# Gancheekim/ATM-VFI

Hardware: AMD Instinct MI355X
Metric: interpolated frames/s at 1080p (network_base, bs=1) (higher is better)
Workload: dtype f32 (contractions as fp16 hi/lo split x3 MFMA, fp32 accumulate; ~22 significand bits)

## Files before the change

### atm-vfi_amd/csrc/api.hip

```cpp
#include "common.h"

#include <string.h>

#include <vector>

namespace atmvfi {

static thread_local char g_err[512] = "";

void set_error(const char* fmt, ...) {
    va_list ap;
    va_start(ap, fmt);
    vsnprintf(g_err, sizeof(g_err), fmt, ap);
    va_end(ap);
}

int check_launch(const char* what) {
    const hipError_t e = hipGetLastError();
    if (e != hipSuccess) {
        set_error("%s: launch failed: %s", what, hipGetErrorString(e));
        return ATMVFI_ELAUNCH;
    }
    return ATMVFI_OK;
}

#ifdef ATMVFI_RANGE_CHECK
static std::vector<RangeWordSetter>& range_registry() {
    static std::vector<RangeWordSetter> v;
    return v;
}
void range_registry_add(RangeWordSetter s) { range_registry().push_back(s); }
#endif

}

extern "C" int atmvfi_range_word_set(uint32_t* word, void* stream) {
#ifdef ATMVFI_RANGE_CHECK
    for (atmvfi::RangeWordSetter set : atmvfi::range_registry()) {
        const int e = set(reinterpret_cast<unsigned*>(word), (hipStream_t)stream);
        ATMVFI_REQUIRE(e == 0, ATMVFI_ELAUNCH, "range_word_set: hipMemcpyToSymbolAsync failed (%d)", e);
    }
    return ATMVFI_OK;
#else
    (void)word; (void)stream;
    atmvfi::set_error("range_word_set: this is the default build; the operand range check lives in libatmvfi_hip_checked.so (make checked)");
    return ATMVFI_EINVAL;
#endif
}
extern "C" int atmvfi_range_checked(void) {
#ifdef ATMVFI_RANGE_CHECK
    return 1;
#else
    return 0;
#endif
}

extern "C" int atmvfi_version(void) { return (0 << 16) | (21 << 8) | 0; }
extern "C" const char* atmvfi_last_error(void) { return atmvfi::g_err; }
#ifndef ATMVFI_SOURCE_DIGEST
#define ATMVFI_SOURCE_DIGEST "unknown (api.hip compiled outside the Makefile)"
#endif
extern "C" const char* atmvfi_source_digest(void) { return ATMVFI_SOURCE_DIGEST; }
```

### atm-vfi_amd/csrc/plan_dispatch.inc

```
#define ATMVFI_PLAN_NFN 65
static const char* const kPlanFnNames[ATMVFI_PLAN_NFN] = {
    "atmvfi_conv2d",
    "atmvfi_conv3x3_f16x3",
    "atmvfi_conv3x3_planes",
    "atmvfi_conv3x3_planes2",
    "atmvfi_conv3x3_planes3",
    "atmvfi_conv3x3_planes_readout",
    "atmvfi_deconv2x2",
    "atmvfi_dwconv3x3_gelu",
    "atmvfi_ensemble_select",
    "atmvfi_f32_to_yuv420p10",
    "atmvfi_final_residual",
    "atmvfi_flow_warp",
    "atmvfi_flow_warp_ex",
    "atmvfi_flow_warp_nhwc",
    "atmvfi_flow_warp_tiled",
    "atmvfi_flow_warp_up2",
    "atmvfi_flow_warp_up2_tiled",
    "atmvfi_frame_borders",
    "atmvfi_frame_compose",
    "atmvfi_frame_difference",
    "atmvfi_frame_f32_to_u8",
    "atmvfi_frame_rot180",
    "atmvfi_frame_signature",
    "atmvfi_frame_u8_to_f32",
    "atmvfi_frame_u8_window",
    "atmvfi_gemm",
    "atmvfi_head1x1_planes",
    "atmvfi_image_pyramid",
    "atmvfi_image_pyramid_pack",
    "atmvfi_l1_mean",
    "atmvfi_layernorm",
    "atmvfi_linear",
    "atmvfi_motion_head",
    "atmvfi_motion_head_planes",
    "atmvfi_pack_dw_weight",
    "atmvfi_pack_frames",
    "atmvfi_pack_weight",
    "atmvfi_pack_weight_conv3x3",
    "atmvfi_pack_weight_split",
    "atmvfi_pool_blocks",
    "atmvfi_range_word_set",
    "atmvfi_refine_tail",
    "atmvfi_resize_bilinear_ac",
    "atmvfi_rgb_to_yuv420",
    "atmvfi_shutter_accumulate",
    "atmvfi_shutter_resolve",
    "atmvfi_split_planes",
    "atmvfi_split_planes_at",
    "atmvfi_ssim_psnr",
    "atmvfi_stem_fused",
    "atmvfi_tta_merge",
    "atmvfi_warp_blend",
    "atmvfi_warp_blend_planes",
    "atmvfi_warp_blend_tiled",
    "atmvfi_window_attention",
    "atmvfi_window_attention_f16x3",
    "atmvfi_window_attn_cross_motion",
    "atmvfi_window_attn_self",
    "atmvfi_yuv420_to_rgb",
    "atmvfi_yuv420_window",
    "atmvfi_yuv420p10_to_f32",
    "atmvfi_yuv_sub_decode",
    "atmvfi_yuv_sub_encode",
    "atmvfi_yuv_surface_decode",
    "atmvfi_yuv_surface_encode",
};
static const int kPlanFnArgs[ATMVFI_PLAN_NFN] = {1, 19, 21, 25, 27, 15, 1, 13, 13, 10, 8, 10, 9, 14, 10, 8, 8, 7, 15, 12, 9, 5, 11, 9, 15, 1, 10, 8, 9, 7, 14, 1, 12, 17, 3, 6, 7, 5, 8, 8, 1, 10, 13, 13, 13, 7, 8, 10, 18, 21, 11, 19, 23, 23, 13, 13, 9, 8, 14, 18, 14, 25, 17, 24, 16};
static int plan_call(const atmvfi_plan_op* op, void* stream) {
    const atmvfi_plan_arg* a = op->a;
    switch (op->fn) {
    case 0: return atmvfi_conv2d((const atmvfi_gemm_params*)(uintptr_t)a[0].u, stream);
    case 1: return atmvfi_conv3x3_f16x3((const float*)(uintptr_t)a[0].u, (int)a[1].i, (int)a[2].i, (int)a[3].i, (int)a[4].i, (int)a[5].i, (const void*)(uintptr_t)a[6].u, (const void*)(uintptr_t)a[7].u, (int)a[8].i, (float*)(uintptr_t)a[9].u, (int)a[10].i, (const float*)(uintptr_t)a[11].u, (const float*)(uintptr_t)a[12].u, (void*)(uintptr_t)a[13].u, (void*)(uintptr_t)a[14].u, (int64_t)a[15].i, (const float*)(uintptr_t)a[16].u, (int)a[17].i, (int)a[18].i, stream);
    case 2: return atmvfi_conv3x3_planes((const void*)(uintptr_t)a[0].u, (const void*)(uintptr_t)a[1].u, (int64_t)a[2].i, (int)a[3].i, (int)a[4].i, (int)a[5].i, (int)a[6].i, (const void*)(uintptr_t)a[7].u, (const void*)(uintptr_t)a[8].u, (int)a[9].i, (float*)(uintptr_t)a[10].u, (int)a[11].i, (const float*)(uintptr_t)a[12].u, (const float*)(uintptr_t)a[13].u, (void*)(uintptr_t)a[14].u, (void*)(uintptr_t)a[15].u, (int64_t)a[16].i, (int)a[17].i, (const float*)(uintptr_t)a[18].u, (int)a[19].i, (int)a[20].i, stream);
    case 3: return atmvfi_conv3x3_planes2((const void*)(uintptr_t)a[0].u, (const void*)(uintptr_t)a[1].u, (int64_t)a[2].i, (int)a[3].i, (int)a[4].i, (int)a[5].i, (int)a[6].i, (const void*)(uintptr_t)a[7].u, (const void*)(uintptr_t)a[8].u, (int)a[9].i, (float*)(uintptr_t)a[10].u, (int)a[11].i, (const float*)(uintptr_t)a[12].u, (const float*)(uintptr_t)a[13].u, (void*)(uintptr_t)a[14].u, (void*)(uintptr_t)a[15].u, (int64_t)a[16].i, (int)a[17].i, (const float*)(uintptr_t)a[18].u, (void*)(uintptr_t)a[19].u, (void*)(uintptr_t)a[20].u, (int64_t)a[21].i, (int)a[22].i, (int)a[23].i, (int)a[24].i, stream);
    case 4: return atmvfi_conv3x3_planes3((const void*)(uintptr_t)a[0].u, (const void*)(uintptr_t)a[1].u, (int64_t)a[2].i, (int)a[3].i, (int)a[4].i, (int)a[5].i, (int)a[6].i, (const void*)(uintptr_t)a[7].u, (const void*)(uintptr_t)a[8].u, (int)a[9].i, (float*)(uintptr_t)a[10].u, (int)a[11].i, (const float*)(uintptr_t)a[12].u, (const float*)(uintptr_t)a[13].u, (void*)(uintptr_t)a[14].u, (void*)(uintptr_t)a[15].u, (int64_t)a[16].i, (int)a[17].i, (const float*)(uintptr_t)a[18].u, (void*)(uintptr_t)a[19].u, (void*)(uintptr_t)a[20].u, (int64_t)a[21].i, (int)a[22].i, (int)a[23].i, (int)a[24].i, (float*)(uintptr_t)a[25].u, (int64_t)a[26].i, stream);
    case 5: return atmvfi_conv3x3_planes_readout((const void*)(uintptr_t)a[0].u, (const void*)(uintptr_t)a[1].u, (int64_t)a[2].i, (int)a[3].i, (int)a[4].i, (int)a[5].i, (int)a[6].i, (const void*)(uintptr_t)a[7].u, (const void*)(uintptr_t)a[8].u, (int)a[9].i, (const float*)(uintptr_t)a[10].u, (const float*)(uintptr_t)a[11].u, (const void*)(uintptr_t)a[12].u, (float*)(uintptr_t)a[13].u, (int64_t)a[14].i, stream);
    case 6: return atmvfi_deconv2x2((const atmvfi_gemm_params*)(uintptr_t)a[0].u, stream);
    case 7: return atmvfi_dwconv3x3_gelu((const float*)(uintptr_t)a[0].u, (int)a[1].i, (float*)(uintptr_t)a[2].u, (int)a[3].i, (const float*)(uintptr_t)a[4].u, (const float*)(uintptr_t)a[5].u, (int)a[6].i, (int)a[7].i, (int)a[8].i, (int)a[9].i, (void*)(uintptr_t)a[10].u, (void*)(uintptr_t)a[11].u, (int)a[12].i, stream);
    case 8: return atmvfi_ensemble_select((const float*)(uintptr_t)a[0].u, (const float*)(uintptr_t)a[1].u, (const float*)(uintptr_t)a[2].u, (const float*)(uintptr_t)a[3].u, (const float*)(uintptr_t)a[4].u, (const float*)(uintptr_t)a[5].u, (const float*)(uintptr_t)a[6].u, (const float*)(uintptr_t)a[7].u, (const float*)(uintptr_t)a[8].u, (float*)(uintptr_t)a[9].u, (float*)(uintptr_t)a[10].u, (int)a[11].i, (int64_t)a[12].i, stream);
    case 9: return atmvfi_f32_to_yuv420p10((const float*)(uintptr_t)a[0].u, (int)a[1].i, (int)a[2].i, (int)a[3].i, (int)a[4].i, (int)a[5].i, (int)a[6].i, (int)a[7].i, (int)a[8].i, (void*)(uintptr_t)a[9].u, stream);
    case 10: return atmvfi_final_residual((const float*)(uintptr_t)a[0].u, (const float*)(uintptr_t)a[1].u, (int)a[2].i, (float*)(uintptr_t)a[3].u, (float*)(uintptr_t)a[4].u, (int)a[5].i, (int)a[6].i, (int)a[7].i, stream);
    case 11: return atmvfi_flow_warp((const float*)(uintptr_t)a[0].u, (const float*)(uintptr_t)a[1].u, (int64_t)a[2].i, (int)a[3].i, (int)a[4].i, (float*)(uintptr_t)a[5].u, (int)a[6].i, (int)a[7].i, (int)a[8].i, (int)a[9].i, stream);
    case 12: return atmvfi_flow_warp_ex((const float*)(uintptr_t)a[0].u, (const float*)(uintptr_t)a[1].u, (float*)(uintptr_t)a[2].u, (uint8_t*)(uintptr_t)a[3].u, (int)a[4].i, (int)a[5].i, (int)a[6].i, (int)a[7].i, (int)a[8].i, stream);
    case 13: return atmvfi_flow_warp_nhwc((const float*)(uintptr_t)a[0].u, (int)a[1].i, (int64_t)a[2].i, (const float*)(uintptr_t)a[3].u, (int64_t)a[4].i, (int)a[5].i, (int)a[6].i, (float*)(uintptr_t)a[7].u, (int)a[8].i, (int64_t)a[9].i, (int)a[10].i, (int)a[11].i, (int)a[12].i, (int)a[13].i, stream);
    case 14: return atmvfi_flow_warp_tiled((const float*)(uintptr_t)a[0].u, (const float*)(uintptr_t)a[1].u, (int64_t)a[2].i, (int)a[3].i, (int)a[4].i, (float*)(uintptr_t)a[5].u, (int)a[6].i, (int)a[7].i, (int)a[8].i, (int)a[9].i, stream);
    case 15: return atmvfi_flow_warp_up2((const float*)(uintptr_t)a[0].u, (const float*)(uintptr_t)a[1].u, (float*)(uintptr_t)a[2].u, (float*)(uintptr_t)a[3].u, (int)a[4].i, (int)a[5].i, (int)a[6].i, (int)a[7].i, stream);
    case 16: return atmvfi_flow_warp_up2_tiled((const float*)(uintptr_t)a[0].u, (const float*)(uintptr_t)a[1].u, (float*)(uintptr_t)a[2].u, (float*)(uintptr_t)a[3].u, (int)a[4].i, (int)a[5].i, (int)a[6].i, (int)a[7].i, stream);
    case 17: return atmvfi_frame_borders((const void*)(uintptr_t)a[0].u, (int)a[1].i, (int)a[2].i, (int)a[3].i, (int32_t*)(uintptr_t)a[4].u, (int32_t*)(uintptr_t)a[5].u, (int64_t)a[6].i, stream);
    case 18: return atmvfi_frame_compose((void*)(uintptr_t)a[0].u, (const void*)(uintptr_t)a[1].u, (int)a[2].i, (int)a[3].i, (int)a[4].i, (int)a[5].i, (int)a[6].i, (int)a[7].i, (const float*)(uintptr_t)a[8].u, (int)a[9].i, (int)a[10].i, (int)a[11].i, (int)a[12].i, (const void*)(uintptr_t)a[13].u, (int)a[14].i, stream);
    case 19: return atmvfi_frame_difference((const void*)(uintptr_t)a[0].u, (const void*)(uintptr_t)a[1].u, (int)a[2].i, (int)a[3].i, (int)a[4].i, (int)a[5].i, (int)a[6].i, (int)a[7].i, (int)a[8].i, (int32_t*)(uintptr_t)a[9].u, (int32_t*)(uintptr_t)a[10].u, (int64_t)a[11].i, stream);
    case 20: return atmvfi_frame_f32_to_u8((const float*)(uintptr_t)a[0].u, (int)a[1].i, (int)a[2].i, (int)a[3].i, (int)a[4].i, (void*)(uintptr_t)a[5].u, (int)a[6].i, (int)a[7].i, (int)a[8].i, stream);
    case 21: return atmvfi_frame_rot180((const float*)(uintptr_t)a[0].u, (float*)(uintptr_t)a[1].u, (int)a[2].i, (int)a[3].i, (int)a[4].i, stream);
    case 22: return atmvfi_frame_signature((const void*)(uintptr_t)a[0].u, (int)a[1].i, (int)a[2].i, (int)a[3].i, (int)a[4].i, (int)a[5].i, (int)a[6].i, (int)a[7].i, (int32_t*)(uintptr_t)a[8].u, (int32_t*)(uintptr_t)a[9].u, (int64_t)a[10].i, stream);
    case 23: return atmvfi_frame_u8_to_f32((const void*)(uintptr_t)a[0].u, (int)a[1].i, (int)a[2].i, (int)a[3].i, (float*)(uintptr_t)a[4].u, (int)a[5].i, (int)a[6].i, (int)a[7].i, (int)a[8].i, stream);
    case 24: return atmvfi_frame_u8_window((const void*)(uintptr_t)a[0].u, (int)a[1].i, (int)a[2].i, (int)a[3].i, (int)a[4].i, (int)a[5].i, (int)a[6].i, (int)a[7].i, (int)a[8].i, (float*)(uintptr_t)a[9].u, (int)a[10].i, (int)a[11].i, (int)a[12].i, (int)a[13].i, (void*)(uintptr_t)a[14].u, stream);
    case 25: return atmvfi_gemm((const atmvfi_gemm_params*)(uintptr_t)a[0].u, stream);
    case 26: return atmvfi_head1x1_planes((const void*)(uintptr_t)a[0].u, (const void*)(uintptr_t)a[1].u, (int64_t)a[2].i, (int64_t)a[3].i, (int)a[4].i, (const float*)(uintptr_t)a[5].u, (const float*)(uintptr_t)a[6].u, (int)a[7].i, (float*)(uintptr_t)a[8].u, (int)a[9].i, stream);
    case 27: return atmvfi_image_pyramid((const float*)(uintptr_t)a[0].u, (const float*)(uintptr_t)a[1].u, (float*)(uintptr_t)a[2].u, (float*)(uintptr_t)a[3].u, (float*)(uintptr_t)a[4].u, (int)a[5].i, (int)a[6].i, (int)a[7].i, stream);
    case 28: return atmvfi_image_pyramid_pack((const float*)(uintptr_t)a[0].u, (const float*)(uintptr_t)a[1].u, (float*)(uintptr_t)a[2].u, (float*)(uintptr_t)a[3].u, (float*)(uintptr_t)a[4].u, (float*)(uintptr_t)a[5].u, (int)a[6].i, (int)a[7].i, (int)a[8].i, stream);
    case 29: return atmvfi_l1_mean((const float*)(uintptr_t)a[0].u, (const float*)(uintptr_t)a[1].u, (float*)(uintptr_t)a[2].u, (int)a[3].i, (int64_t)a[4].i, (float*)(uintptr_t)a[5].u, (int64_t)a[6].i, stream);
    case 30: return atmvfi_layernorm((const float*)(uintptr_t)a[0].u, (int)a[1].i, (int64_t)a[2].i, (int)a[3].i, (const int32_t*)(uintptr_t)a[4].u, (float*)(uintptr_t)a[5].u, (int)a[6].i, (const float*)(uintptr_t)a[7].u, (const float*)(uintptr_t)a[8].u, (int64_t)a[9].i, (int)a[10].i, (void*)(uintptr_t)a[11].u, (void*)(uintptr_t)a[12].u, (int)a[13].i, stream);
    case 31: return atmvfi_linear((const atmvfi_gemm_params*)(uintptr_t)a[0].u, stream);
    case 32: return atmvfi_motion_head((const float*)(uintptr_t)a[0].u, (const int32_t*)(uintptr_t)a[1].u, (const float*)(uintptr_t)a[2].u, (const float*)(uintptr_t)a[3].u, (const float*)(uintptr_t)a[4].u, (const float*)(uintptr_t)a[5].u, (float*)(uintptr_t)a[6].u, (int)a[7].i, (int64_t)a[8].i, (int)a[9].i, (int64_t)a[10].i, (int)a[11].i, stream);
    case 33: return atmvfi_motion_head_planes((const float*)(uintptr_t)a[0].u, (const int32_t*)(uintptr_t)a[1].u, (const float*)(uintptr_t)a[2].u, (const float*)(uintptr_t)a[3].u, (const float*)(uintptr_t)a[4].u, (const float*)(uintptr_t)a[5].u, (float*)(uintptr_t)a[6].u, (int)a[7].i, (int64_t)a[8].i, (int)a[9].i, (int64_t)a[10].i, (int)a[11].i, (void*)(uintptr_t)a[12].u, (void*)(uintptr_t)a[13].u, (int64_t)a[14].i, (int)a[15].i, (int)a[16].i, stream);
    case 34: return atmvfi_pack_dw_weight((const float*)(uintptr_t)a[0].u, (float*)(uintptr_t)a[1].u, (int)a[2].i, stream);
    case 35: return atmvfi_pack_frames((const float*)(uintptr_t)a[0].u, (const float*)(uintptr_t)a[1].u, (float*)(uintptr_t)a[2].u, (int)a[3].i, (int)a[4].i, (int)a[5].i, stream);
    case 36: return atmvfi_pack_weight((int)a[0].i, (const float*)(uintptr_t)a[1].u, (float*)(uintptr_t)a[2].u, (int)a[3].i, (int)a[4].i, (int)a[5].i, (int)a[6].i, stream);
    case 37: return atmvfi_pack_weight_conv3x3((const float*)(uintptr_t)a[0].u, (void*)(uintptr_t)a[1].u, (void*)(uintptr_t)a[2].u, (int)a[3].i, (int)a[4].i, stream);
    case 38: return atmvfi_pack_weight_split((int)a[0].i, (const float*)(uintptr_t)a[1].u, (void*)(uintptr_t)a[2].u, (void*)(uintptr_t)a[3].u, (int)a[4].i, (int)a[5].i, (int)a[6].i, (int)a[7].i, stream);
    case 39: return atmvfi_pool_blocks((void*)(uintptr_t)a[0].u, (int64_t)a[1].i, (int)a[2].i, (const int32_t*)(uintptr_t)a[3].u, (int)a[4].i, (int64_t)a[5].i, (void*)(uintptr_t)a[6].u, (int)a[7].i, stream);
    case 40: return atmvfi_range_word_set((uint32_t*)(uintptr_t)a[0].u, stream);
    case 41: return atmvfi_refine_tail((const float*)(uintptr_t)a[0].u, (int64_t)a[1].i, (const float*)(uintptr_t)a[2].u, (const float*)(uintptr_t)a[3].u, (const float*)(uintptr_t)a[4].u, (float*)(uintptr_t)a[5].u, (float*)(uintptr_t)a[6].u, (int)a[7].i, (int)a[8].i, (int)a[9].i, stream);
    case 42: return atmvfi_resize_bilinear_ac((const float*)(uintptr_t)a[0].u, (int64_t)a[1].i, (int64_t)a[2].i, (int64_t)a[3].i, (int64_t)a[4].i, (float*)(uintptr_t)a[5].u, (int)a[6].i, (int)a[7].i, (int)a[8].i, (int)a[9].i, (int)a[10].i, (int)a[11].i, (float)a[12].f, stream);
    case 43: return atmvfi_rgb_to_yuv420((const void*)(uintptr_t)a[0].u, (int)a[1].i, (const float*)(uintptr_t)a[2].u, (int)a[3].i, (int)a[4].i, (int)a[5].i, (int)a[6].i, (int)a[7].i, (int)a[8].i, (int)a[9].i, (int)a[10].i, (int)a[11].i, (void*)(uintptr_t)a[12].u, stream);
    case 44: return atmvfi_shutter_accumulate((int32_t*)(uintptr_t)a[0].u, (int)a[1].i, (int)a[2].i, (const float*)(uintptr_t)a[3].u, (int)a[4].i, (int)a[5].i, (int)a[6].i, (int)a[7].i, (const uint8_t*)(uintptr_t)a[8].u, (int)a[9].i, (int)a[10].i, (int)a[11].i, (int)a[12].i, stream);
    case 45: return atmvfi_shutter_resolve((const int32_t*)(uintptr_t)a[0].u, (int)a[1].i, (int)a[2].i, (int)a[3].i, (int)a[4].i, (uint8_t*)(uintptr_t)a[5].u, (int)a[6].i, stream);
    case 46: return atmvfi_split_planes((const float*)(uintptr_t)a[0].u, (int)a[1].i, (int64_t)a[2].i, (int)a[3].i, (const float*)(uintptr_t)a[4].u, (void*)(uintptr_t)a[5].u, (void*)(uintptr_t)a[6].u, (int)a[7].i, stream);
    case 47: return atmvfi_split_planes_at((const float*)(uintptr_t)a[0].u, (int)a[1].i, (int64_t)a[2].i, (int)a[3].i, (const float*)(uintptr_t)a[4].u, (void*)(uintptr_t)a[5].u, (void*)(uintptr_t)a[6].u, (int)a[7].i, (int)a[8].i, (int)a[9].i, stream);
    case 48: return atmvfi_ssim_psnr((const void*)(uintptr_t)a[0].u, (int64_t)a[1].i, (int64_t)a[2].i, (int64_t)a[3].i, (int64_t)a[4].i, (const float*)(uintptr_t)a[5].u, (int64_t)a[6].i, (int64_t)a[7].i, (int64_t)a[8].i, (int64_t)a[9].i, (int)a[10].i, (int)a[11].i, (int)a[12].i, (float)a[13].f, (int)a[14].i, (double*)(uintptr_t)a[15].u, (float*)(uintptr_t)a[16].u, (int64_t)a[17].i, stream);
    case 49: return atmvfi_stem_fused((const float*)(uintptr_t)a[0].u, (int)a[1].i, (int)a[2].i, (int)a[3].i, (int)a[4].i, (int)a[5].i, (const void*)(uintptr_t)a[6].u, (const void*)(uintptr_t)a[7].u, (const float*)(uintptr_t)a[8].u, (const float*)(uintptr_t)a[9].u, (const void*)(uintptr_t)a[10].u, (const void*)(uintptr_t)a[11].u, (const float*)(uintptr_t)a[12].u, (const float*)(uintptr_t)a[13].u, (const void*)(uintptr_t)a[14].u, (const void*)(uintptr_t)a[15].u, (const float*)(uintptr_t)a[16].u, (const float*)(uintptr_t)a[17].u, (void*)(uintptr_t)a[18].u, (void*)(uintptr_t)a[19].u, (int64_t)a[20].i, stream);
    case 50: return atmvfi_tta_merge((const float*)(uintptr_t)a[0].u, (const float*)(uintptr_t)a[1].u, (float*)(uintptr_t)a[2].u, (void*)(uintptr_t)a[3].u, (int)a[4].i, (int)a[5].i, (int)a[6].i, (int)a[7].i, (int)a[8].i, (int)a[9].i, (int)a[10].i, stream);
    case 51: return atmvfi_warp_blend((const float*)(uintptr_t)a[0].u, (const float*)(uintptr_t)a[1].u, (const float*)(uintptr_t)a[2].u, (int)a[3].i, (int64_t)a[4].i, (float*)(uintptr_t)a[5].u, (float*)(uintptr_t)a[6].u, (float*)(uintptr_t)a[7].u, (float*)(uintptr_t)a[8].u, (float*)(uintptr_t)a[9].u, (float*)(uintptr_t)a[10].u, (float*)(uintptr_t)a[11].u, (const float*)(uintptr_t)a[12].u, (const float*)(uintptr_t)a[13].u, (float*)(uintptr_t)a[14].u, (int)a[15].i, (int)a[16].i, (int)a[17].i, (int)a[18].i, stream);
    case 52: return atmvfi_warp_blend_planes((const float*)(uintptr_t)a[0].u, (const float*)(uintptr_t)a[1].u, (const float*)(uintptr_t)a[2].u, (int)a[3].i, (int64_t)a[4].i, (float*)(uintptr_t)a[5].u, (float*)(uintptr_t)a[6].u, (float*)(uintptr_t)a[7].u, (float*)(uintptr_t)a[8].u, (float*)(uintptr_t)a[9].u, (float*)(uintptr_t)a[10].u, (float*)(uintptr_t)a[11].u, (const float*)(uintptr_t)a[12].u, (const float*)(uintptr_t)a[13].u, (float*)(uintptr_t)a[14].u, (int)a[15].i, (void*)(uintptr_t)a[16].u, (void*)(uintptr_t)a[17].u, (int64_t)a[18].i, (int)a[19].i, (int)a[20].i, (int)a[21].i, (int)a[22].i, stream);
    case 53: return atmvfi_warp_blend_tiled((const float*)(uintptr_t)a[0].u, (const float*)(uintptr_t)a[1].u, (const float*)(uintptr_t)a[2].u, (int)a[3].i, (int64_t)a[4].i, (float*)(uintptr_t)a[5].u, (float*)(uintptr_t)a[6].u, (float*)(uintptr_t)a[7].u, (float*)(uintptr_t)a[8].u, (float*)(uintptr_t)a[9].u, (float*)(uintptr_t)a[10].u, (float*)(uintptr_t)a[11].u, (const float*)(uintptr_t)a[12].u, (const float*)(uintptr_t)a[13].u, (float*)(uintptr_t)a[14].u, (int)a[15].i, (void*)(uintptr_t)a[16].u, (void*)(uintptr_t)a[17].u, (int64_t)a[18].i, (int)a[19].i, (int)a[20].i, (int)a[21].i, (int)a[22].i, stream);
    case 54: return atmvfi_window_attention((const float*)(uintptr_t)a[0].u, (float*)(uintptr_t)a[1].u, (float*)(uintptr_t)a[2].u, (const int32_t*)(uintptr_t)a[3].u, (int)a[4].i, (int)a[5].i, (int)a[6].i, (int)a[7].i, (int)a[8].i, (int)a[9].i, (void*)(uintptr_t)a[10].u, (void*)(uintptr_t)a[11].u, (int)a[12].i, stream);
    case 55: return atmvfi_window_attention_f16x3((const float*)(uintptr_t)a[0].u, (float*)(uintptr_t)a[1].u, (float*)(uintptr_t)a[2].u, (const int32_t*)(uintptr_t)a[3].u, (int)a[4].i, (int)a[5].i, (int)a[6].i, (int)a[7].i, (int)a[8].i, (int)a[9].i, (void*)(uintptr_t)a[10].u, (void*)(uintptr_t)a[11].u, (int)a[12].i, stream);
    case 56: return atmvfi_window_attn_cross_motion((const float*)(uintptr_t)a[0].u, (float*)(uintptr_t)a[1].u, (float*)(uintptr_t)a[2].u, (const int32_t*)(uintptr_t)a[3].u, (int)a[4].i, (int)a[5].i, (int)a[6].i, (int)a[7].i, (int)a[8].i, stream);
    case 57: return atmvfi_window_attn_self((const float*)(uintptr_t)a[0].u, (float*)(uintptr_t)a[1].u, (const int32_t*)(uintptr_t)a[2].u, (int)a[3].i, (int)a[4].i, (int)a[5].i, (int)a[6].i, (int)a[7].i, stream);
    case 58: return atmvfi_yuv420_to_rgb((const void*)(uintptr_t)a[0].u, (int)a[1].i, (int)a[2].i, (int)a[3].i, (int)a[4].i, (int)a[5].i, (int)a[6].i, (void*)(uintptr_t)a[7].u, (int)a[8].i, (float*)(uintptr_t)a[9].u, (int)a[10].i, (int)a[11].i, (int)a[12].i, (int)a[13].i, stream);
    case 59: return atmvfi_yuv420_window((const void*)(uintptr_t)a[0].u, (int)a[1].i, (int)a[2].i, (int)a[3].i, (int)a[4].i, (int)a[5].i, (int)a[6].i, (int)a[7].i, (int)a[8].i, (int)a[9].i, (int)a[10].i, (int)a[11].i, (float*)(uintptr_t)a[12].u, (int)a[13].i, (int)a[14].i, (int)a[15].i, (int)a[16].i, (void*)(uintptr_t)a[17].u, stream);
    case 60: return atmvfi_yuv420p10_to_f32((const void*)(uintptr_t)a[0].u, (int)a[1].i, (int)a[2].i, (int)a[3].i, (int)a[4].i, (int)a[5].i, (int)a[6].i, (int)a[7].i, (int)a[8].i, (float*)(uintptr_t)a[9].u, (int)a[10].i, (int)a[11].i, (int)a[12].i, (int)a[13].i, stream);
    case 61: return atmvfi_yuv_sub_decode((const void*)(uintptr_t)a[0].u, (int)a[1].i, (int)a[2].i, (int)a[3].i, (int)a[4].i, (int)a[5].i, (int)a[6].i, (int)a[7].i, (int)a[8].i, (int)a[9].i, (int64_t)a[10].i, (int64_t)a[11].i, (int64_t)a[12].i, (int)a[13].i, (int)a[14].i, (int)a[15].i, (int)a[16].i, (int)a[17].i, (void*)(uintptr_t)a[18].u, (int)a[19].i, (float*)(uintptr_t)a[20].u, (int)a[21].i, (int)a[22].i, (int)a[23].i, (int)a[24].i, stream);
    case 62: return atmvfi_yuv_sub_encode((const void*)(uintptr_t)a[0].u, (int)a[1].i, (const float*)(uintptr_t)a[2].u, (int)a[3].i, (int)a[4].i, (int)a[5].i, (int)a[6].i, (int)a[7].i, (int)a[8].i, (int)a[9].i, (int)a[10].i, (int)a[11].i, (int)a[12].i, (int)a[13].i, (int)a[14].i, (int)a[15].i, (void*)(uintptr_t)a[16].u, stream);
    case 63: return atmvfi_yuv_surface_decode((const void*)(uintptr_t)a[0].u, (int)a[1].i, (int)a[2].i, (int)a[3].i, (int)a[4].i, (int)a[5].i, (int)a[6].i, (int)a[7].i, (int)a[8].i, (int64_t)a[9].i, (int64_t)a[10].i, (int64_t)a[11].i, (int)a[12].i, (int)a[13].i, (int)a[14].i, (int)a[15].i, (int)a[16].i, (void*)(uintptr_t)a[17].u, (int)a[18].i, (float*)(uintptr_t)a[19].u, (int)a[20].i, (int)a[21].i, (int)a[22].i, (int)a[23].i, stream);
    case 64: return atmvfi_yuv_surface_encode((const void*)(uintptr_t)a[0].u, (int)a[1].i, (const float*)(uintptr_t)a[2].u, (int)a[3].i, (int)a[4].i, (int)a[5].i, (int)a[6].i, (int)a[7].i, (int)a[8].i, (int)a[9].i, (int)a[10].i, (int)a[11].i, (int)a[12].i, (int)a[13].i, (int)a[14].i, (void*)(uintptr_t)a[15].u, stream);
    default: break;
    }
    atmvfi::set_error("plan_run: unknown function id %d", op->fn);
    return ATMVFI_EINVAL;
}
```

### atm-vfi_amd/hip_ops.py

```python
from __future__ import annotations

import ctypes
import os
from dataclasses import dataclass
from typing import List, Optional

import torch

from .pixfmt import Surface, _not_420, _origin_error, as_surface

_HERE = os.path.dirname(os.path.abspath(__file__))
LIB_PATH = os.path.join(_HERE, "libatmvfi_hip.so")
CHECKED_LIB_PATH = os.path.join(_HERE, "libatmvfi_hip_checked.so")

GEMM_CONV, GEMM_LINEAR, GEMM_DECONV = 0, 1, 2

c_f = ctypes.c_void_p
c_i = ctypes.c_int
C_SLOTS = ctypes.POINTER(ctypes.c_int32)
c_l = ctypes.c_int64


class HipLibraryMissing(RuntimeError):
    pass


class GemmParams(ctypes.Structure):
    _fields_ = [
        ("mode", ctypes.c_int32),
        ("in_", c_f), ("in_ld", ctypes.c_int32), ("N", ctypes.c_int32), ("H", ctypes.c_int32),
        ("W", ctypes.c_int32), ("Cin", ctypes.c_int32),
        ("in_gstride", ctypes.c_int64), ("in_rpg", ctypes.c_int32),
        ("weight", c_f),
        ("Cout", ctypes.c_int32), ("kh", ctypes.c_int32), ("kw", ctypes.c_int32), ("stride", ctypes.c_int32),
        ("pad", ctypes.c_int32), ("dil", ctypes.c_int32),
        ("Ho", ctypes.c_int32), ("Wo", ctypes.c_int32),
        ("M", ctypes.c_int64),
        ("out", c_f), ("out_ld", ctypes.c_int32),
        ("out_gstride", ctypes.c_int64), ("out_rpg", ctypes.c_int32),
        ("out_row_map", c_f),
        ("bias", c_f), ("prelu", c_f), ("in_prelu", c_f), ("residual", c_f),
        ("res_ld", ctypes.c_int32),
        ("precision", ctypes.c_int32), ("weight_hi", c_f), ("weight_lo", c_f),
        ("in_hi", c_f), ("in_lo", c_f),
        ("out_hi", c_f), ("out_lo", c_f), ("out_plane_rows", ctypes.c_int64), ("out_plane_c0", ctypes.c_int32),
        ("out_plane_gc", ctypes.c_int32), ("tile_wn", ctypes.c_int32),
        ("in_hi2", c_f), ("in_lo2", c_f), ("in_ld2", ctypes.c_int32), ("in_split_chunks", ctypes.c_int32),
        ("workspace", c_f), ("workspace_floats", ctypes.c_int64),
    ]


class PlanArg(ctypes.Union):
    _fields_ = [("u", ctypes.c_uint64), ("i", ctypes.c_int64), ("f", ctypes.c_double)]


PLAN_MAX_ARGS = 28


class PlanOp(ctypes.Structure):
    _fields_ = [("fn", ctypes.c_int32), ("nargs", ctypes.c_int32), ("a", PlanArg * PLAN_MAX_ARGS)]


class PlanPatch(ctypes.Structure):
    _fields_ = [("op", ctypes.c_int32), ("arg", ctypes.c_int32), ("slot", ctypes.c_int32), ("reserved", ctypes.c_int32),
                ("offset", ctypes.c_int64)]


SIGNATURES = {
    "atmvfi_version": (c_i, []),
    "atmvfi_last_error": (ctypes.c_char_p, []),
    "atmvfi_source_digest": (ctypes.c_char_p, []),
    "atmvfi_range_word_set": (c_i, [c_f, c_f]),
    "atmvfi_range_checked": (c_i, []),
    "atmvfi_gemm": (c_i, [ctypes.POINTER(GemmParams), c_f]),
    "atmvfi_gemm_workspace_floats": (c_l, [c_l, c_i, c_i]),
    "atmvfi_split_planes": (c_i, [c_f, c_i, c_l, c_i, c_f, c_f, c_f, c_i, c_f]),
    "atmvfi_split_planes_at": (c_i, [c_f, c_i, c_l, c_i, c_f, c_f, c_f, c_i, c_i, c_i, c_f]),
    "atmvfi_conv2d": (c_i, [ctypes.POINTER(GemmParams), c_f]),
    "atmvfi_linear": (c_i, [ctypes.POINTER(GemmParams), c_f]),
    "atmvfi_deconv2x2": (c_i, [ctypes.POINTER(GemmParams), c_f]),
    "atmvfi_packed_weight_floats": (c_l, [c_i, c_i, c_i, c_i, c_i]),
    "atmvfi_pack_weight": (c_i, [c_i, c_f, c_f, c_i, c_i, c_i, c_i, c_f]),
    "atmvfi_split_weight_halves": (c_l, [c_i, c_i, c_i, c_i, c_i]),
    "atmvfi_pack_weight_split": (c_i, [c_i, c_f, c_f, c_f, c_i, c_i, c_i, c_i, c_f]),
    "atmvfi_conv3x3_weight_halves": (c_l, [c_i, c_i]),
    "atmvfi_pack_weight_conv3x3": (c_i, [c_f, c_f, c_f, c_i, c_i, c_f]),
    "atmvfi_conv3x3_f16x3": (c_i, [c_f, c_i, c_i, c_i, c_i, c_i, c_f, c_f, c_i, c_f, c_i, c_f, c_f, c_f, c_f, c_l, c_f, c_i, c_i, c_f]),
    "atmvfi_conv3x3_planes": (c_i, [c_f, c_f, c_l, c_i, c_i, c_i, c_i, c_f, c_f, c_i, c_f, c_i, c_f, c_f, c_f, c_f, c_l, c_i, c_f, c_i, c_i, c_f]),
    "atmvfi_flow_warp_up2": (c_i, [c_f, c_f, c_f, c_f, c_i, c_i, c_i, c_i, c_f]),
    "atmvfi_flow_warp_up2_tiled": (c_i, [c_f, c_f, c_f, c_f, c_i, c_i, c_i, c_i, c_f]),
    "atmvfi_image_pyramid": (c_i, [c_f, c_f, c_f, c_f, c_f, c_i, c_i, c_i, c_f]),
    "atmvfi_image_pyramid_pack": (c_i, [c_f, c_f, c_f, c_f, c_f, c_f, c_i, c_i, c_i, c_f]),
    "atmvfi_head1x1_planes": (c_i, [c_f, c_f, c_l, c_l, c_i, c_f, c_f, c_i, c_f, c_i, c_f]),
    "atmvfi_conv3x3_planes2": (c_i, [c_f, c_f, c_l, c_i, c_i, c_i, c_i, c_f, c_f, c_i, c_f, c_i, c_f, c_f, c_f, c_f, c_l, c_i, c_f, c_f, c_f, c_l, c_i, c_i, c_i, c_f]),
    "atmvfi_conv3x3_planes3": (c_i, [c_f, c_f, c_l, c_i, c_i, c_i, c_i, c_f, c_f, c_i, c_f, c_i, c_f, c_f, c_f, c_f, c_l, c_i, c_f, c_f, c_f, c_l, c_i, c_i, c_i, c_f, c_l, c_f]),
    "atmvfi_conv3x3_planes_workspace_floats": (c_l, [c_i, c_i, c_i, c_i, c_i]),
    "atmvfi_conv3x3_planes_readout": (c_i, [c_f, c_f, c_l, c_i, c_i, c_i, c_i, c_f, c_f, c_i, c_f, c_f, c_f, c_f, c_l, c_f]),
    "atmvfi_refine_tail": (c_i, [c_f, c_l, c_f, c_f, c_f, c_f, c_f, c_i, c_i, c_i, c_f]),
    "atmvfi_layernorm": (c_i, [c_f, c_i, c_l, c_i, c_f, c_f, c_i, c_f, c_f, c_l, c_i, c_f, c_f, c_i, c_f]),
    "atmvfi_dwconv3x3_gelu": (c_i, [c_f, c_i, c_f, c_i, c_f, c_f, c_i, c_i, c_i, c_i, c_f, c_f, c_i, c_f]),
    "atmvfi_pack_dw_weight": (c_i, [c_f, c_f, c_i, c_f]),
    "atmvfi_window_attention": (c_i, [c_f, c_f, c_f, c_f, c_i, c_i, c_i, c_i, c_i, c_i, c_f, c_f, c_i, c_f]),
    "atmvfi_window_attention_f16x3": (c_i, [c_f, c_f, c_f, c_f, c_i, c_i, c_i, c_i, c_i, c_i, c_f, c_f, c_i, c_f]),
    "atmvfi_window_attn_cross_motion": (c_i, [c_f, c_f, c_f, c_f, c_i, c_i, c_i, c_i, c_i, c_f]),
    "atmvfi_window_attn_self": (c_i, [c_f, c_f, c_f, c_i, c_i, c_i, c_i, c_i, c_f]),
    "atmvfi_motion_head": (c_i, [c_f, c_f, c_f, c_f, c_f, c_f, c_f, c_i, c_l, c_i, c_l, c_i, c_f]),
    "atmvfi_motion_head_planes": (c_i, [c_f, c_f, c_f, c_f, c_f, c_f, c_f, c_i, c_l, c_i, c_l, c_i, c_f, c_f, c_l, c_i, c_i, c_f]),
    "atmvfi_flow_warp": (c_i, [c_f, c_f, c_l, c_i, c_i, c_f, c_i, c_i, c_i, c_i, c_f]),
    "atmvfi_flow_warp_tiled": (c_i, [c_f, c_f, c_l, c_i, c_i, c_f, c_i, c_i, c_i, c_i, c_f]),
    "atmvfi_flow_warp_ex": (c_i, [c_f, c_f, c_f, c_f, c_i, c_i, c_i, c_i, c_i, c_f]),
    "atmvfi_flow_warp_nhwc": (c_i, [c_f, c_i, c_l, c_f, c_l, c_i, c_i, c_f, c_i, c_l, c_i, c_i, c_i, c_i, c_f]),
    "atmvfi_warp_blend": (c_i, [c_f, c_f, c_f, c_i, c_l, c_f, c_f, c_f, c_f, c_f, c_f, c_f, c_f, c_f, c_f, c_i,
                                c_i, c_i, c_i, c_f]),
    "atmvfi_warp_blend_planes": (c_i, [c_f, c_f, c_f, c_i, c_l, c_f, c_f, c_f, c_f, c_f, c_f, c_f, c_f, c_f, c_f, c_i,
                                       c_f, c_f, c_l, c_i, c_i, c_i, c_i, c_f]),
    "atmvfi_warp_blend_tiled": (c_i, [c_f, c_f, c_f, c_i, c_l, c_f, c_f, c_f, c_f, c_f, c_f, c_f, c_f, c_f, c_f, c_i,
                                      c_f, c_f, c_l, c_i, c_i, c_i, c_i, c_f]),
    "atmvfi_resize_bilinear_ac": (c_i, [c_f, c_l, c_l, c_l, c_l, c_f, c_i, c_i, c_i, c_i, c_i, c_i, ctypes.c_float, c_f]),
    "atmvfi_frame_u8_to_f32": (c_i, [c_f, c_i, c_i, c_i, c_f, c_i, c_i, c_i, c_i, c_f]),
    "atmvfi_frame_u8_window": (c_i, [c_f, c_i, c_i, c_i, c_i, c_i, c_i, c_i, c_i, c_f, c_i, c_i, c_i, c_i, c_f, c_f]),
    "atmvfi_frame_f32_to_u8": (c_i, [c_f, c_i, c_i, c_i, c_i, c_f, c_i, c_i, c_i, c_f]),
    "atmvfi_pool_blocks": (c_i, [c_f, c_l, c_i, C_SLOTS, c_i, c_l, c_f, c_i, c_f]),
    "atmvfi_tta_merge": (c_i, [c_f, c_f, c_f, c_f, c_i, c_i, c_i, c_i, c_i, c_i, c_i, c_f]),
    "atmvfi_frame_rot180": (c_i, [c_f, c_f, c_i, c_i, c_i, c_f]),
    "atmvfi_frame_signature_workspace_ints": (c_l, [c_i, c_i]),
    "atmvfi_frame_signature": (c_i, [c_f, c_i, c_i, c_i, c_i, c_i, c_i, c_i, c_f, c_f, c_l, c_f]),
    "atmvfi_frame_difference_workspace_ints": (c_l, [c_i, c_i]),
    "atmvfi_frame_difference": (c_i, [c_f, c_f, c_i, c_i, c_i, c_i, c_i, c_i, c_i, c_f, c_f, c_l, c_f]),
    "atmvfi_frame_borders_workspace_ints": (c_l, [c_i, c_i]),
    "atmvfi_frame_borders": (c_i, [c_f, c_i, c_i, c_i, c_f, c_f, c_l, c_f]),
    "atmvfi_frame_compose": (c_i, [c_f, c_f, c_i, c_i, c_i, c_i, c_i, c_i, c_f, c_i, c_i, c_i, c_i, c_f, c_i, c_f]),
    "atmvfi_shutter_accumulate": (c_i, [c_f, c_i, c_i, c_f, c_i, c_i, c_i, c_i, c_f, c_i, c_i, c_i, c_i, c_f]),
    "atmvfi_shutter_resolve": (c_i, [c_f, c_i, c_i, c_i, c_i, c_f, c_i, c_f]),
    "atmvfi_shutter_table": (c_i, [c_i, ctypes.POINTER(ctypes.c_uint16)]),
    "atmvfi_yuv420_to_rgb": (c_i, [c_f, c_i, c_i, c_i, c_i, c_i, c_i, c_f, c_i, c_f, c_i, c_i, c_i, c_i, c_f]),
    "atmvfi_yuv420_window": (c_i, [c_f, c_i, c_i, c_i, c_i, c_i, c_i, c_i, c_i, c_i, c_i, c_i, c_f, c_i, c_i, c_i, c_i, c_f, c_f]),
    "atmvfi_rgb_to_yuv420": (c_i, [c_f, c_i, c_f, c_i, c_i, c_i, c_i, c_i, c_i, c_i, c_i, c_i, c_f, c_f]),
    "atmvfi_yuv420p10_to_f32": (c_i, [c_f, c_i, c_i, c_i, c_i, c_i, c_i, c_i, c_i, c_f, c_i, c_i, c_i, c_i, c_f]),
    "atmvfi_f32_to_yuv420p10": (c_i, [c_f, c_i, c_i, c_i, c_i, c_i, c_i, c_i, c_i, c_f, c_f]),
    "atmvfi_yuv_surface_decode": (c_i, [c_f, c_i, c_i, c_i, c_i, c_i, c_i, c_i, c_i, c_l, c_l, c_l, c_i, c_i, c_i, c_i, c_i, c_f, c_i, c_f, c_i, c_i,
                                        c_i, c_i, c_f]),
    "atmvfi_yuv_surface_encode": (c_i, [c_f, c_i, c_f, c_i, c_i, c_i, c_i, c_i, c_i, c_i, c_i, c_i, c_i, c_i, c_i, c_f, c_f]),
    "atmvfi_yuv_sub_decode": (c_i, [c_f, c_i, c_i, c_i, c_i, c_i, c_i, c_i, c_i, c_i, c_l, c_l, c_l, c_i, c_i, c_i, c_i, c_i, c_f, c_i, c_f, c_i, c_i,
                                    c_i, c_i, c_f]),
    "atmvfi_yuv_sub_encode": (c_i, [c_f, c_i, c_f, c_i, c_i, c_i, c_i, c_i, c_i, c_i, c_i, c_i, c_i, c_i, c_i, c_i, c_f, c_f]),
    "atmvfi_pack_frames": (c_i, [c_f, c_f, c_f, c_i, c_i, c_i, c_f]),
    "atmvfi_final_residual": (c_i, [c_f, c_f, c_i, c_f, c_f, c_i, c_i, c_i, c_f]),
    "atmvfi_l1_mean": (c_i, [c_f, c_f, c_f, c_i, c_l, c_f, c_l, c_f]),
    "atmvfi_l1_mean_workspace_floats": (c_l, [c_i, c_l]),
    "atmvfi_ssim_psnr": (c_i, [c_f, c_l, c_l, c_l, c_l, c_f, c_l, c_l, c_l, c_l, c_i, c_i, c_i, ctypes.c_float, c_i, c_f, c_f, c_l, c_f]),
    "atmvfi_ssim_psnr_workspace_floats": (c_l, [c_i, c_i, c_i]),
    "atmvfi_ensemble_select": (c_i, [c_f, c_f, c_f, c_f, c_f, c_f, c_f, c_f, c_f, c_f, c_f, c_i, c_l, c_f]),
    "atmvfi_stem_fused": (c_i, [c_f, c_i, c_i, c_i, c_i, c_i, c_f, c_f, c_f, c_f, c_f, c_f, c_f, c_f, c_f, c_f, c_f, c_f, c_f, c_f, c_l, c_f]),
    "atmvfi_plan_fn_id": (c_i, [ctypes.c_char_p]),
    "atmvfi_plan_run": (c_i, [ctypes.POINTER(PlanOp), c_i, ctypes.POINTER(PlanPatch), c_i, ctypes.POINTER(ctypes.c_uint64), c_i,
                              ctypes.POINTER(c_i), c_f]),
}
SSIM_X_U8, SSIM_X_BGR, SSIM_ROUND_Y, SSIM_ACCUMULATE, SSIM_MSE_F32 = 1, 2, 4, 8, 16


def load_library(path: str = LIB_PATH) -> ctypes.CDLL:
    if not os.path.exists(path):
        raise HipLibraryMissing(
            f"{path} not found: build it with `python -c 'import __graft_entry__ as g; g.build()'` "
            "(hipcc --offload-arch=gfx950).  There is no CPU fallback.")
    lib = ctypes.CDLL(path)
    for name, (res, args) in SIGNATURES.items():
        fn = getattr(lib, name)
        fn.restype = res
        fn.argtypes = args
    return lib


@dataclass
class PackedWeight:
    mode: int
    cout: int
    cin: int
    kh: int
    kw: int
    orig: torch.Tensor
    packed: Optional[torch.Tensor]
    hi: Optional[torch.Tensor] = None
    lo: Optional[torch.Tensor] = None
    hi3: Optional[torch.Tensor] = None
    lo3: Optional[torch.Tensor] = None


@dataclass
class StemWeights:
    c0: int
    c1: int
    w1h: torch.Tensor
    w1l: torch.Tensor
    b1: torch.Tensor
    p1: torch.Tensor
    w2h: torch.Tensor
    w2l: torch.Tensor
    b2: torch.Tensor
    p2: torch.Tensor
    w3h: torch.Tensor
    w3l: torch.Tensor
    b3: torch.Tensor
    p3: torch.Tensor


class Planes:

    def __init__(self, t: torch.Tensor, c: int, rows: Optional[int] = None):
        if t.dtype != torch.float16 or t.dim() != 4 or t.shape[0] != 2 or t.shape[3] != 32 or not t.is_contiguous() or c > t.shape[1] * 32 \
                or c <= (t.shape[1] - 1) * 32:
            raise ValueError(f"Planes: expected contiguous fp16 [2, ceil(C/32), rows, 32], got {tuple(t.shape)} {t.dtype} C={c}")
        if not t.is_cuda:
            raise TypeError("Planes: tensor must live on the GPU")
        if rows is not None and not 0 < rows <= t.shape[2]:
            raise ValueError(f"Planes: {rows} valid rows do not fit the {t.shape[2]} allocated ones")
        self.t, self.c = t, c
        self._rows = t.shape[2] if rows is None else rows

    @property
    def rows(self):
        return self._rows

    @property
    def ld_rows(self):
        return self.t.shape[2]

    @property
    def chunks(self):
        return self.t.shape[1]

    def to_rows(self) -> torch.Tensor:
        return self.t[:, :, :self.rows].permute(0, 2, 1, 3).reshape(2, self.rows, self.chunks * 32)

    def to_float(self) -> torch.Tensor:
        r = self.to_rows().float()
        return (r[0] + r[1] / 1024.0)[:, :self.c]

    @staticmethod
    def alloc(rows: int, c: int, device) -> "Planes":
        return Planes(torch.zeros(2, (c + 31) // 32, rows + 1, 32, dtype=torch.float16, device=device), c, rows)


class TPtr(ctypes.c_void_p):
    __slots__ = ("src",)


def _ptr(t: Optional[torch.Tensor], byte_offset: int = 0):
    if t is None:
# ... 488 lines not shown
                           w3h, w3l, b3.detach().float().contiguous(), p3.detach().float().contiguous())

    def stem_fused(self, x, w: "StemWeights", out: Planes):
        _chk(x, "stem_fused.x")
        if x.dim() != 4 or x.shape[3] != 4 or not x.is_contiguous():
            raise ValueError(f"stem_fused: expected contiguous NHWC4 frames [F,H,W,4], got {tuple(x.shape)}")
        f, h, wd, _ = x.shape
        if h % 2 or wd % 2 or out.rows != f * (h // 2) * (wd // 2) or out.c != w.c1:
            raise ValueError(f"stem_fused: planes [{out.rows},{out.c}] do not hold {f}x{h // 2}x{wd // 2} pixels x {w.c1} channels")
        if self.precision != "f16x3":
            raise ValueError("stem_fused: needs the f16x3 engine")
        flops = 2.0 * f * h * wd * (27 * w.c0 + 9 * w.c0 * w.c0) + 2.0 * f * (h // 2) * (wd // 2) * 9 * w.c0 * w.c1
        meta = {"flops": flops, "bytes": 16.0 * f * h * wd + 4.0 * out.rows * out.chunks * 32, "shape": f"{f}x{h}x{wd} 3>{w.c0}>{w.c0}>{w.c1}s2"}
        self._run("stem_fused", meta, self.lib.atmvfi_stem_fused, _ptr(x), f, h, wd, w.c0, w.c1, _ptr(w.w1h), _ptr(w.w1l), _ptr(w.b1), _ptr(w.p1),
                  _ptr(w.w2h), _ptr(w.w2l), _ptr(w.b2), _ptr(w.p2), _ptr(w.w3h), _ptr(w.w3l), _ptr(w.b3), _ptr(w.p3),
                  _ptr(out.t[0]), _ptr(out.t[1]), out.ld_rows, self._stream())

    def conv3x3_planes(self, x: Planes, n: int, h: int, wd: int, w: PackedWeight, out=None, bias=None, prelu=None,
                       planes: Optional[Planes] = None, planes_c0: int = 0, planes_prelu=None, in_chunk0: int = 0, cin: Optional[int] = None,
                       wn: int = 0, out_cmin: int = 0, planes2: Optional[Planes] = None, planes2_c0: int = 0,
                       workspace: Optional[torch.Tensor] = None):
        cin = (x.c - 32 * in_chunk0) if cin is None else cin
        if self.precision != "f16x3" or w.hi3 is None:
            raise ValueError("conv3x3_planes: needs the f16x3 engine and the conv3x3 weight planes")
        if w.mode != GEMM_CONV or w.kh != 3 or w.kw != 3 or w.cin != cin:
            raise ValueError(f"conv3x3_planes: weight ({w.cout},{w.cin},{w.kh},{w.kw}) does not match Cin {cin}")
        if x.rows != n * h * wd or x.ld_rows <= x.rows or 32 * in_chunk0 + cin > x.chunks * 32:
            raise ValueError(f"conv3x3_planes: input planes [{x.rows} (+{x.ld_rows - x.rows} spare), {x.c}] do not fit {n}x{h}x{wd} pixels x {cin} channels "
                             "(one spare zero row is required)")
        cout = w.cout
        old = 0
        out_ptr = _ptr(out)
        if out is not None:
            old, on, oh, ow, oc = nhwc_view(out, "conv3x3_planes.out")
            if (on, oh, ow) == (n, h, wd) and oc == cout - out_cmin and out_cmin > 0:
                out_ptr = _ptr(out, -4 * out_cmin)
            elif (on, oh, ow, oc) != (n, h, wd, cout):
                raise ValueError(f"conv3x3_planes: out {tuple(out.shape)} != [{n},{h},{wd},{cout}] (or {cout - out_cmin} channels: compact)")
        elif planes is None:
            raise ValueError("conv3x3_planes: no output")
        if planes is not None:
            if planes.rows != n * h * wd or planes_c0 % 8 or planes_c0 + cout > planes.chunks * 32:
                raise ValueError(f"conv3x3_planes: plane sink [{planes.rows},{planes.c}] cannot take {cout} channels at offset {planes_c0}")
            if planes_prelu is not None and planes_prelu.numel() < (cout + 31) // 32 * 32:
                raise ValueError("conv3x3_planes: planes_prelu must be padded to a multiple of 32 channels")
        if planes2 is not None and (planes is None or planes2.rows != n * h * wd or planes2_c0 % 8 or planes2_c0 + cout > planes2.chunks * 32):
            raise ValueError(f"conv3x3_planes: second plane sink [{planes2.rows},{planes2.c}] needs the first one and room for {cout} channels at {planes2_c0}")
        meta = {"flops": 2.0 * n * h * wd * cout * cin * 9, "bytes": 4.0 * (n * h * wd * (cin + cout) + cout * cin * 9),
                "shape": f"M{n * h * wd} N{cout} K{cin * 9}"}
        coff = in_chunk0 * x.ld_rows * 32 * 2
        if workspace is not None and (workspace.dtype != torch.float32 or not workspace.is_cuda or not workspace.is_contiguous()):
            raise ValueError("conv3x3_planes: the split-K workspace must be a contiguous CUDA fp32 tensor")
        self._run("conv3x3_planes", meta, self.lib.atmvfi_conv3x3_planes3, _ptr(x.t[0], coff), _ptr(x.t[1], coff), x.ld_rows,
                  n, h, wd, cin, _ptr(w.hi3), _ptr(w.lo3), cout, out_ptr, old, _ptr(bias), _ptr(prelu),
                  _ptr(planes.t[0]) if planes is not None else None, _ptr(planes.t[1]) if planes is not None else None,
                  planes.ld_rows if planes is not None else 0, planes_c0, _ptr(planes_prelu) if planes is not None else None,
                  _ptr(planes2.t[0]) if planes2 is not None else None, _ptr(planes2.t[1]) if planes2 is not None else None,
                  planes2.ld_rows if planes2 is not None else 0, planes2_c0, out_cmin, wn, _ptr(workspace),
                  workspace.numel() if workspace is not None else 0, self._stream())

    def pack_readout(self, w: torch.Tensor) -> torch.Tensor:
        o3, c, kh, kw = w.shape
        if (o3, kh, kw) != (3, 3, 3) or c not in (32, 64):
            raise ValueError(f"pack_readout: expected a [3, 32 | 64, 3, 3] weight, got {tuple(w.shape)}")
        w2 = torch.zeros(32, c, dtype=torch.float32, device=self.device)
        w2[:27] = w.detach().float().permute(2, 3, 0, 1).reshape(27, c)
        kk_n = c // 32
        lane = torch.arange(64, device=self.device)
        r, g = lane & 15, lane >> 4
        cb = 8 * (g & 1) + 4 * (g >> 1)
        e = torch.arange(8, device=self.device)
        ch = cb[:, None] + torch.where(e < 4, e, 16 + e - 4)[None, :]
        full = torch.empty(2, kk_n, 64, 8, dtype=torch.float32, device=self.device)
        for t in range(2):
            for kk in range(kk_n):
                full[t, kk] = w2[(16 * t + r)[:, None].expand(64, 8), 32 * kk + ch]
        hi = full.half()
        lo = ((full - hi.float()) * 1024.0).half()
        return torch.stack([hi, lo], 0).contiguous()

    def conv3x3_planes_readout(self, x: Planes, n: int, h: int, wd: int, w: PackedWeight, bias, prelu, w2: torch.Tensor, contrib: torch.Tensor):
        if self.precision != "f16x3" or w.hi3 is None or w.kh != 3 or w.cin > x.chunks * 32 or x.rows != n * h * wd or x.ld_rows <= x.rows:
            raise ValueError("conv3x3_planes_readout: needs the f16x3 engine, conv3x3 weight planes and input planes with a spare zero row")
        if w.cout not in (32, 64) or tuple(w2.shape) != (2, 2, w.cout // 32, 64, 8) or w2.dtype != torch.float16:
            raise ValueError("conv3x3_planes_readout: Cout must be 32 or 64 and w2 the pack_readout() operand of that width")
        if contrib.dtype != torch.float32 or contrib.dim() != 2 or contrib.shape[0] != 27 or contrib.shape[1] < n * h * wd or not contrib.is_contiguous():
            raise ValueError("conv3x3_planes_readout: contrib must be contiguous fp32 [27, >= N*H*W]")
        meta = {"flops": 2.0 * n * h * wd * w.cout * (w.cin * 9 + 27), "bytes": 4.0 * n * h * wd * (w.cin + 27), "shape": f"M{n * h * wd} N{w.cout} K{w.cin * 9} +27"}
        self._run("conv3x3_planes", meta, self.lib.atmvfi_conv3x3_planes_readout, _ptr(x.t[0]), _ptr(x.t[1]), x.ld_rows, n, h, wd, w.cin,
                  _ptr(w.hi3), _ptr(w.lo3), w.cout, _ptr(bias), _ptr(prelu), _ptr(w2), _ptr(contrib), contrib.shape[1], self._stream())

    def refine_tail(self, contrib, bias, slope, it, it_sum, it_clamped):
        _planar(it, 3, "refine_tail.it"); _planar(it_sum, 3, "refine_tail.sum"); _planar(it_clamped, 3, "refine_tail.clamped")
        b, _, h, w = it.shape
        if contrib.dim() != 2 or contrib.shape[0] != 27 or contrib.shape[1] < b * h * w or not contrib.is_contiguous():
            raise ValueError("refine_tail: contrib must be contiguous fp32 [27, >= B*H*W]")
        self._run("refine_tail", {"bytes": 4.0 * b * h * w * (27 + 9)}, self.lib.atmvfi_refine_tail, _ptr(contrib), contrib.shape[1], _ptr(bias),
                  _ptr(slope), _ptr(it), _ptr(it_sum), _ptr(it_clamped), b, h, w, self._stream())

    def conv3x3_workspace_floats(self, n: int, h: int, wd: int, cin: int, cout: int) -> int:
        return int(self.lib.atmvfi_conv3x3_planes_workspace_floats(n, h, wd, cin, cout))

    def head1x1_planes(self, x: Planes, n: int, h: int, wd: int, w: PackedWeight, out, bias=None):
        old, on, oh, ow, oc = nhwc_view(out, "head1x1_planes.out")
        if w.mode != GEMM_CONV or w.kh != 1 or w.cout > 8 or (on, oh, ow, oc) != (n, h, wd, w.cout) or x.rows != n * h * wd or w.cin > x.chunks * 32:
            raise ValueError(f"head1x1_planes: weight ({w.cout},{w.cin},{w.kh},{w.kw}) / out {tuple(out.shape)} / planes [{x.rows},{x.c}] mismatch")
        wt = w.orig.detach()
        if not wt.is_contiguous():
            wt = wt.contiguous()
        meta = {"flops": 2.0 * n * h * wd * w.cout * w.cin, "bytes": 4.0 * n * h * wd * (w.cin + w.cout), "shape": f"M{n * h * wd} N{w.cout} K{w.cin}"}
        self._run("head1x1_planes", meta, self.lib.atmvfi_head1x1_planes, _ptr(x.t[0]), _ptr(x.t[1]), x.ld_rows, n * h * wd, w.cin,
                  _ptr(wt), _ptr(bias), w.cout, _ptr(out), old, self._stream())

    def conv_planes(self, x: Planes, n: int, h: int, wd: int, w: PackedWeight, out=None, stride=1, pad=1, dil=1, bias=None, prelu=None,
                    sink: Optional[Planes] = None, sink_c0: int = 0, in_chunk0: int = 0, x2: Optional[Planes] = None, x2_chunk0: int = 0,
                    split_chunks: int = 0):
        if self.precision != "f16x3" or w.hi is None or w.mode != GEMM_CONV:
            raise ValueError("conv_planes: needs the f16x3 engine and split conv weights")
        cin, cout = w.cin, w.cout
        oh = (h + 2 * pad - dil * (w.kh - 1) - 1) // stride + 1
        ow = (wd + 2 * pad - dil * (w.kw - 1) - 1) // stride + 1
        c1 = 32 * split_chunks if x2 is not None else cin
        for t, c0, cc, what in ((x, in_chunk0, c1, "x"),) + (((x2, x2_chunk0, cin - c1, "x2"),) if x2 is not None else ()):
            if t.rows != n * h * wd or t.ld_rows <= t.rows or 32 * c0 + cc > t.chunks * 32:
                raise ValueError(f"conv_planes: {what} [{t.rows} (+{t.ld_rows - t.rows} spare), {t.c}] does not hold {n}x{h}x{wd} pixels x "
                                 f"{cc} channels from chunk {c0} (one spare zero row is required)")
        if x2 is not None and not 0 < 32 * split_chunks < cin:
            raise ValueError("conv_planes: split_chunks must cut the input channels at a 32-channel boundary inside (0, Cin)")
        old = 0
        if out is not None:
            old, on, ooh, oow, oc = nhwc_view(out, "conv_planes.out")
            if (on, ooh, oow, oc) != (n, oh, ow, cout):
                raise ValueError(f"conv_planes: out {tuple(out.shape)} != [{n},{oh},{ow},{cout}]")
        elif sink is None:
            raise ValueError("conv_planes: no output")
        p = GemmParams(mode=GEMM_CONV, in_=None, in_ld=x.ld_rows, N=n, H=h, W=wd, Cin=cin, in_gstride=0, in_rpg=0,
                       weight=w.packed.data_ptr(), Cout=cout, kh=w.kh, kw=w.kw, stride=stride, pad=pad, dil=dil,
                       Ho=oh, Wo=ow, M=n * oh * ow, out=None if out is None else out.data_ptr(), out_ld=old, out_gstride=0, out_rpg=0,
                       out_row_map=None, bias=_ptr(bias), prelu=_ptr(prelu), in_prelu=None, residual=None, res_ld=0)
        p.precision, p.weight_hi, p.weight_lo = 1, w.hi.data_ptr(), w.lo.data_ptr()
        off = in_chunk0 * x.ld_rows * 64
        p.in_hi, p.in_lo = x.t[0].data_ptr() + off, x.t[1].data_ptr() + off
        if x2 is not None:
            off2 = x2_chunk0 * x2.ld_rows * 64
            p.in_hi2, p.in_lo2, p.in_ld2, p.in_split_chunks = x2.t[0].data_ptr() + off2, x2.t[1].data_ptr() + off2, x2.ld_rows, split_chunks
        p.tile_wn = self.gemm_tile_wn if self.gemm_tile_wn < 0 else 0
        self._gemm_sink(p, sink, n * oh * ow, cout, sink_c0, 0, 1, "conv_planes")
        meta = {"flops": 2.0 * n * oh * ow * cout * cin * w.kh * w.kw, "bytes": 4.0 * (n * h * wd * cin + n * oh * ow * cout + cout * cin * w.kh * w.kw),
                "shape": f"M{n * oh * ow} N{cout} K{cin * w.kh * w.kw}"}
        ws = self._gemm_splitk(p, n * oh * ow, cout, w.kh * w.kw * ((cin + 31) // 32))
        p._srcs = (out, bias, prelu, ws)
        self._run("conv2d_split", meta, self.lib.atmvfi_conv2d, ctypes.byref(p), self._stream())

    def deconv(self, x, w: PackedWeight, out, bias=None, prelu=None, in_prelu=None, planes: Optional[Planes] = None,
               sink: Optional[Planes] = None, sink_c0: int = 0, in_shape=None):
        if x is None:
            if planes is None or in_shape is None:
                raise ValueError("deconv: no input")
            ld, (n, h, wd, cin) = 0, in_shape
        else:
            ld, n, h, wd, cin = nhwc_view(x, "deconv.in")
        cout = w.cout
        if out is None:
            if sink is None:
                raise ValueError("deconv: no output")
            old, on, oh, ow = 0, n, 2 * h, 2 * wd
        else:
            old, on, oh, ow, oc = nhwc_view(out, "deconv.out")
            if oc != cout:
                raise ValueError(f"deconv: out has {oc} channels, weight {cout}")
        if cin != w.cin or on != n or w.mode != GEMM_DECONV or oh != 2 * h or ow != 2 * wd:
            raise ValueError(f"deconv: shape mismatch in {(n, h, wd, cin)} w ({w.cin},{w.cout}) out {(on, oh, ow, cout)}")
        p = GemmParams(mode=GEMM_DECONV, in_=None if x is None else x.data_ptr(), in_ld=ld, N=n, H=h, W=wd, Cin=cin, in_gstride=0, in_rpg=0,
                       weight=w.packed.data_ptr(), Cout=cout, kh=2, kw=2, stride=2, pad=0, dil=1, Ho=oh, Wo=ow,
                       M=n * h * wd, out=None if out is None else out.data_ptr(), out_ld=old, out_gstride=0, out_rpg=0, out_row_map=None,
                       bias=_ptr(bias), prelu=_ptr(prelu), in_prelu=_ptr(in_prelu), residual=None, res_ld=0)
        p.precision, p.weight_hi, p.weight_lo = self._prec(w)
        p.tile_wn = self.gemm_tile_wn
        self._gemm_sink(p, sink, n * oh * ow, cout, sink_c0, 0, 1, "deconv")
        use_planes = planes is not None and p.precision == 1
        if x is None and not use_planes:
            raise ValueError("deconv: plane input needs the f16x3 engine")
        if use_planes:
            if planes.rows < n * h * wd or planes.c != cin:
                raise ValueError("deconv: planes do not match the input rows")
            p.in_, p.in_ld, p.in_prelu = None, planes.ld_rows, None
            p.in_hi, p.in_lo = planes.t[0].data_ptr(), planes.t[1].data_ptr()
        meta = {"flops": 2.0 * n * h * wd * 4 * cout * cin, "bytes": 4.0 * (n * h * wd * cin + n * oh * ow * cout + 4 * cout * cin),
                "shape": f"M{n * h * wd} N{4 * cout} K{cin}"}
        ws = self._gemm_splitk(p, n * h * wd, 4 * ((cout + 3) // 4 * 4), (cin + 31) // 32) if use_planes else None
        p._srcs = (x, out, bias, prelu, in_prelu, ws)
        self._run("deconv2x2_split" if use_planes else "deconv2x2_f16x3" if p.precision else "deconv2x2", meta, self.lib.atmvfi_deconv2x2,
                  ctypes.byref(p), self._stream())

    split_planes_ok = True
    pyramid_packs = True
    motion_head_sink = True

    def split_planes(self, x, out: Planes, prelu=None, c0: Optional[int] = None):
        ld, m, c, gs, _ = rows_view(x, "split_planes.in")
        if gs != 0 or m != out.rows or (c0 is None and c != out.c) or (c0 is not None and (c0 % 8 or c0 + c > out.chunks * 32)):
            raise ValueError("split_planes: expected a plain [rows,C] view matching the planes")
        if prelu is not None and prelu.numel() < c:
            raise ValueError("split_planes: prelu needs one slope per channel")
        meta = {"bytes": 4.0 * m * c + 4.0 * m * ((c + 31) // 32 * 32 if c0 is None else (c + 7) // 8 * 8)}
        if c0 is None:
            self._run("split_planes", meta, self.lib.atmvfi_split_planes, _ptr(x), ld, m, c, _ptr(prelu), _ptr(out.t[0]),
                      _ptr(out.t[1]), out.ld_rows, self._stream())
        else:
            self._run("split_planes", meta, self.lib.atmvfi_split_planes_at, _ptr(x), ld, m, c, _ptr(prelu), _ptr(out.t[0]),
                      _ptr(out.t[1]), out.ld_rows, c0, 8, self._stream())

    def linear(self, x, w: PackedWeight, out, bias=None, residual=None, out_row_map=None, sink: Optional[Planes] = None,
               sink_c0: int = 0, sink_gc: int = 0):
        planes = x if isinstance(x, Planes) else None
        if planes is not None:
            if self.precision != "f16x3" or w.hi is None:
                raise ValueError("linear: split-plane input needs the f16x3 engine and split weights")
            ld, m, cin, gs, rpg = planes.ld_rows, planes.rows, planes.c, 0, 0
        else:
            ld, m, cin, gs, rpg = rows_view(x, "linear.in")
        old, mo, cout, ogs, orpg = rows_view(out, "linear.out")
        if cin != w.cin or cout != w.cout or w.kh != 1 or w.mode == GEMM_DECONV:
            raise ValueError(f"linear: shape mismatch in {tuple(x.shape)} w ({w.cout},{w.cin}) out {tuple(out.shape)}")
        if out_row_map is None and mo != m:
            raise ValueError("linear: row count mismatch")
        if out_row_map is not None and (out_row_map.numel() != m or out_row_map.dtype != torch.int32 or not out_row_map.is_cuda):
            raise ValueError("linear: out_row_map must be a CUDA int32 tensor with one entry per GEMM row")
        res_ld = 0
        if residual is not None:
            res_ld, rm, rc, rgs, _ = rows_view(residual, "linear.residual")
            if rm != m or rc != cout or rgs != 0:
                raise ValueError("linear: residual must be a plain [M,Cout] view")
        p = GemmParams(mode=GEMM_LINEAR, in_=None if planes is not None else x.data_ptr(), in_ld=ld, N=1, H=1, W=1, Cin=cin, in_gstride=gs, in_rpg=rpg,
                       weight=w.packed.data_ptr(), Cout=cout, kh=1, kw=1, stride=1, pad=0, dil=1, Ho=1, Wo=1, M=m,
                       out=out.data_ptr(), out_ld=old, out_gstride=ogs, out_rpg=orpg, out_row_map=_ptr(out_row_map),
                       bias=_ptr(bias), prelu=None, in_prelu=None, residual=_ptr(residual), res_ld=res_ld)
        p.precision, p.weight_hi, p.weight_lo = self._prec(w)
        p.tile_wn = self.gemm_tile_wn
        if planes is not None:
            p.in_hi, p.in_lo = planes.t[0].data_ptr(), planes.t[1].data_ptr()
        if sink is not None:
            self._gemm_sink(p, sink, orpg if orpg else mo, cout, sink_c0, sink_gc, (mo // orpg) if orpg else 1, "linear")
        meta = {"flops": 2.0 * m * cout * cin, "bytes": 4.0 * (m * cin + m * cout + cout * cin), "shape": f"M{m} N{cout} K{cin}"}
        ws = self._gemm_splitk(p, m, cout, (cin + 31) // 32) if planes is not None else None
        p._srcs = (None if planes is not None else x, out, bias, residual, out_row_map, ws)
        self._run("linear_split" if planes is not None else "linear_f16x3" if p.precision else "linear", meta, self.lib.atmvfi_linear, ctypes.byref(p), self._stream())

    @staticmethod
    def _sink(planes: Optional[Planes], rows: int, c: int, what: str):
        if planes is None:
            return None, None, 0
        if planes.rows != rows or planes.c != c:
            raise ValueError(f"{what}: planes hold {planes.rows} x {planes.c}, kernel writes {rows} x {c}")
        return _ptr(planes.t[0]), _ptr(planes.t[1]), planes.ld_rows

    def layernorm(self, x, out, gamma, beta, src_row_map=None, planes: Optional[Planes] = None):
        ld, m, c, gs, rpg = rows_view(x, "layernorm.in")
        if out is None:
            if planes is None:
                raise ValueError("layernorm: no output")
            old, mo, co, ogs = 0, planes.rows, planes.c, 0
        else:
            old, mo, co, ogs, _ = rows_view(out, "layernorm.out")
        if co != c or ogs != 0:
            raise ValueError("layernorm: output must be a plain [rows,C] view")
        if src_row_map is None and mo != m:
            raise ValueError("layernorm: row count mismatch")
        if src_row_map is not None and src_row_map.numel() != mo:
            raise ValueError("layernorm: src_row_map needs one entry per output row")
        hi, lo, pld = self._sink(planes, mo, c, "layernorm")
        meta = {"bytes": 4.0 * mo * c * (1 + (out is not None) + (planes is not None))}
        self._run("layernorm", meta, self.lib.atmvfi_layernorm, _ptr(x), ld, gs, rpg, _ptr(src_row_map), _ptr(out), old,
                  _ptr(gamma), _ptr(beta), mo, c, hi, lo, pld, self._stream())

    def dwconv_gelu(self, x, out, w9, bias, planes: Optional[Planes] = None):
        ld, n, h, w, c = nhwc_view(x, "dwconv.in")
        old = 0
        if out is not None:
            old, on, oh, ow, oc = nhwc_view(out, "dwconv.out")
            if (on, oh, ow, oc) != (n, h, w, c):
                raise ValueError("dwconv: shape mismatch")
        elif planes is None:
            raise ValueError("dwconv: no output")
        hi, lo, pld = self._sink(planes, n * h * w, c, "dwconv")
        meta = {"bytes": 4.0 * n * h * w * c * (1 + (out is not None) + (planes is not None))}
        self._run("dwconv3x3_gelu", meta, self.lib.atmvfi_dwconv3x3_gelu, _ptr(x), ld, _ptr(out), old, _ptr(w9), _ptr(bias),
                  n, h, w, c, hi, lo, pld, self._stream())

    def window_attention(self, qkv, out, motion, labels, bw, nw, ws, heads, hd, kv_shift, planes: Optional[Planes] = None):
        _chk(qkv, "attn.qkv")
        n = ws * ws
        c = heads * hd
        if out is None and planes is None:
            raise ValueError("window_attention: no output")
        if out is not None:
            _chk(out, "attn.out")
        if tuple(qkv.shape) != (bw * n, 3 * c) or not qkv.is_contiguous() or (
                out is not None and (tuple(out.shape) != (bw * n, c) or not out.is_contiguous())):
            raise ValueError(f"window_attention: qkv {tuple(qkv.shape)} / out do not match Bw {bw} N {n} C {c}")
        if motion is not None and (tuple(motion.shape) != (bw * n, heads, 2) or not motion.is_contiguous()):
            raise ValueError("window_attention: motion must be contiguous [Bw*N, heads, 2]")
        if labels is not None and (tuple(labels.shape) != (nw, n) or labels.dtype != torch.int32 or not labels.is_cuda):
            raise ValueError("window_attention: labels must be CUDA int32 [nW, N]")
        meta = {"flops": 4.0 * bw * heads * n * n * hd, "bytes": 4.0 * bw * n * 4 * c}
        hi, lo, pld = self._sink(planes, bw * n, c, "window_attention")
# ... 569 lines not shown
```

### atm-vfi_amd/network.py

```python
from __future__ import annotations

import math
import operator
from typing import Dict, List, Optional, Tuple

import torch
import torch.nn as nn

from . import schema as S
from .hip_ops import GEMM_CONV, GEMM_DECONV, GEMM_LINEAR, HipOps, PackedWeight, Planes, PlanUnsupported
from .windows import WindowGeometry, build_window_geometry


_VERSION_OF = operator.attrgetter("_version")
_DATA_PTR_OF = torch.Tensor.data_ptr


_PARAM_EPOCH = [0]


class _ParamWatch:

    def __setattr__(self, name, value):
        d = self.__dict__
# ... 335 lines not shown

    def _apply(self, fn, *a, **k):
        self._plist = None
        return super()._apply(fn, *a, **k)

    def load_state_dict(self, *a, **k):
        self._plist = None
        return super().load_state_dict(*a, **k)

    def invalidate_weights(self):
        self._plist = None
        self._prepared_sig = None

    def _param_sig(self):
        pl = self._plist
        if pl is None or self._pepoch != _PARAM_EPOCH[0]:
            self._pepoch = _PARAM_EPOCH[0]
            pl = self._plist = [p for _, p in self.named_parameters()]
        return (tuple(map(_DATA_PTR_OF, pl)), tuple(map(_VERSION_OF, pl)), tuple(map(id, pl)))

    _RUNTIME_RESET = {"_ops_obj": None, "_prepared_sig": None, "_ws_key": None, "_graph_sig": None, "_plan_sig": None, "_plist": None,
                      "_pepoch": -1, "_frame_cache": None, "_primary": None, "_prepare_lock": None, "_reuse_first": False}
    _RUNTIME_DICTS = ("_bufs", "_geo", "_prepared", "_workspaces", "_graphs", "_plans", "_pool_plans", "_splitk_memo")

    def __getstate__(self):
        d = dict(self.__dict__)
        d.update(self._RUNTIME_RESET)
        for k in self._RUNTIME_DICTS:
            d[k] = {}
        return d

    def __setstate__(self, state):
        super().__setstate__(state)
        _PARAM_EPOCH[0] += 1

    def replica(self) -> "Network":
        import copy
        rep = copy.copy(self)
        rep._ops_obj = None
        object.__setattr__(rep, "_primary", self if self._primary is None else self._primary)
        if rep._primary.__dict__.get("_prepare_lock") is None:
            import threading
            object.__setattr__(rep._primary, "_prepare_lock", threading.Lock())
        rep.local_motion_args = dict(self.local_motion_args)
        rep.global_motion_args = dict(self.global_motion_args)
        rep._prepared, rep._prepared_sig = {}, None
        rep._workspaces, rep._ws_key, rep._bufs, rep._geo = {}, None, {}, {}
        rep._graphs, rep._graph_sig, rep._plans, rep._plan_sig = {}, None, {}, None
        rep._pool_plans, rep._splitk_memo, rep._plan_stats = {}, {}, self._new_plan_stats()
        rep._frame_cache_on, rep._frame_cache, rep._reuse_first = False, None, False
        rep._plist, rep._pepoch = None, -1
        return rep

    def _prepare(self, ops):
        if self._primary is not None:
            pm = self._primary
            with pm._prepare_lock:
                before = pm._prepared_sig
                P = pm._prepare_unlocked(pm._ops(ops.device) if isinstance(ops, HipOps) else ops)
                if pm._prepared_sig is not before and isinstance(ops, HipOps):
                    torch.cuda.current_stream(ops.device).synchronize()
                self._prepared, self._prepared_sig, self._plist = P, pm._prepared_sig, pm._plist
            return P
        lock = self._prepare_lock
        if lock is None:
            return self._prepare_unlocked(ops)
        with lock:
            return self._prepare_unlocked(ops)

    def _prepare_unlocked(self, ops):
        sig = self._param_sig()
        if sig == self._prepared_sig:
            return self._prepared
        sd = {k: v for k, v in self.named_parameters()}
        P: Dict[str, object] = {}
        for k, p in sd.items():
            P[k] = p.detach()
        for sp in S.param_schema(self._v):
            k, shp = sp.key, sp.shape
            if sp.is_buffer or not k.endswith(".weight"):
                continue
            w = sd[k].detach()
            if len(shp) == 4 and "dwconv" in k:
                P["pk:" + k] = ops.pack_dw_weight(w)
            elif len(shp) == 4 and shp[2] == 2:
                P["pk:" + k] = ops.pack_weight(GEMM_DECONV, w)
            elif len(shp) == 4 and shp[2] == 1 and ".proj." in k:
                P["pk:" + k] = ops.pack_weight(GEMM_LINEAR, w.reshape(shp[0], shp[1]))
            elif len(shp) == 4:
                P["pk:" + k] = ops.pack_weight(GEMM_CONV, w)
            elif len(shp) == 2 and ".attn.mlp." not in k:
                if k.endswith("attn.kv.weight"):
                    continue
                if k.endswith("attn.q.weight"):
                    kv = sd[k.replace(".q.weight", ".kv.weight")].detach()
                    P["pk:" + k.replace(".q.weight", ".qkv.weight")] = ops.pack_weight(GEMM_LINEAR, torch.cat([w, kv], 0))
                else:
                    P["pk:" + k] = ops.pack_weight(GEMM_LINEAR, w)
        w3 = self._v.decoder_widths[2] + S.MOTION_OUT
        gap = (-w3) % 8
        if getattr(ops, "split_planes_ok", False):
            wp = sd["proj.0.weight"].detach()
            wpp = torch.cat([wp[:, :w3], torch.zeros(wp.shape[0], gap, 3, 3, dtype=wp.dtype, device=wp.device), wp[:, w3:]], 1)
            P["pk:proj.0.weight:planes"] = ops.pack_weight(GEMM_CONV, wpp.contiguous())
        if hasattr(ops, "pack_readout") and getattr(ops, "split_planes_ok", False):
            P["readout"] = ops.pack_readout(sd["refine_head.1.0.weight"].detach())
        if hasattr(ops, "pack_stem") and getattr(ops, "split_planes_ok", False):
            P["stem"] = ops.pack_stem(*(sd[f"feat_extracts.{a}.{b}"].detach() for a in ("0.0", "0.1", "1.0") for b in ("0.weight", "0.bias", "1.weight")))
        if isinstance(ops, HipOps):
            wmax = float(torch.stack([sd[sp.key].detach().abs().max() for sp in S.param_schema(self._v)
                                      if not sp.is_buffer and sp.key.endswith(".weight") and len(sp.shape) >= 2]).max())
            self.weight_abs_max = wmax
            if wmax > 16384.0:
                import warnings
                warnings.warn(f"atm-vfi_amd: largest |weight| of this checkpoint is {wmax:.0f}; the f16x3 engines saturate operands at "
                              "65504 -- check Network.f16x3_deviation(im0, im1) or use set_precision('f32')")
        for st in (1, 2):
            P[f"inprelu:{st}"] = ops.pad_channels(sd[f"upsample_pyramid.{st}.0.weight"])
        self._prepared = P
        self._prepared_sig = sig
        return P

    def _conv_act(self, ops, P, p, x, out, stride=1):
        ops.conv(x, P[f"pk:{p}.0.weight"], out, stride=stride, pad=1, dil=1, bias=P[f"{p}.0.bias"], prelu=P[f"{p}.1.weight"])

    def _conv_plain(self, ops, P, p, x, out, stride=1, pad=1, dil=1, planes=None, planes_prelu=None):
        if planes is not None:
            ops.conv(x, P[f"pk:{p}.weight"], out, stride=stride, pad=pad, dil=dil, bias=P[f"{p}.bias"], planes=planes,
                     planes_prelu=planes_prelu)
            return
        ops.conv(x, P[f"pk:{p}.weight"], out, stride=stride, pad=pad, dil=dil, bias=P[f"{p}.bias"])

    def _plane_convs(self, ops) -> bool:
        return self._plane_deconvs(ops) and self._rows_fit_planes

    def _c3p(self, ops, P, p, xp, n, h, w, out=None, act=True, sink=None, sink_c0=0, sink_prelu=None, wkey=None, out_cmin=0, sink2=None):
        if act:
            wk, bias, prelu = wkey or f"pk:{p}.0.weight", P[f"{p}.0.bias"], P[f"{p}.1.weight"]
        else:
            wk, bias, prelu = wkey or f"pk:{p}.weight", P[f"{p}.bias"], None
        extra = {} if sink2 is None else {"planes2": sink2}
        need = ops.conv3x3_workspace_floats(n, h, w, P[wk].cin, P[wk].cout)
        if need:
            extra["workspace"] = self.buf("splitk_ws", need)
        ops.conv3x3_planes(xp, n, h, w, P[wk], out=out, bias=bias, prelu=prelu, planes=sink, planes_c0=sink_c0, planes_prelu=sink_prelu,
                           out_cmin=out_cmin, **extra)

    def _conv_p(self, ops, P, p, src: "_PMap", stride=1, pad=1, dil=1, act=True, out=None, sink=None, sink_c0=0, src2: "Optional[_PMap]" = None):
        if act:
            wk, bias, prelu = f"pk:{p}.0.weight", P[f"{p}.0.bias"], P[f"{p}.1.weight"]
        else:
            wk, bias, prelu = f"pk:{p}.weight", P[f"{p}.bias"], None
        two = {} if src2 is None else {"x2": src2.p, "x2_chunk0": src2.chunk0, "split_chunks": src.c // 32}
        ops.conv_planes(src.p, src.n, src.h, src.w, P[wk], out=out, stride=stride, pad=pad, dil=dil, bias=bias, prelu=prelu, sink=sink,
                        sink_c0=sink_c0, in_chunk0=src.chunk0, **two)

    def _deconv_act(self, ops, P, p, x, out, in_prelu=None, split: Optional[str] = None, planes=None):
        w = P[f"pk:{p}.0.weight"]
        if planes is not None:
            ops.deconv(x, w, out, bias=P[f"{p}.0.bias"], prelu=P[f"{p}.1.weight"], planes=planes)
            return
        if split is not None and self._plane_deconvs(ops) and w.hi is not None:
            b, h, wd, cin = x.shape
            xp = self.planes(split, b * h * wd, cin)
            ops.split_planes(x.flatten(0, 2), xp, prelu=in_prelu)
            ops.deconv(x, w, out, bias=P[f"{p}.0.bias"], prelu=P[f"{p}.1.weight"], planes=xp)
            return
        ops.deconv(x, w, out, bias=P[f"{p}.0.bias"], prelu=P[f"{p}.1.weight"], in_prelu=in_prelu)

    def _encoder(self, ops, P, x0, tag: str):
        d = self._v.hidden_dims
        f, h, w, _ = x0.shape
        if self._plane_convs(ops):
            ld = self._v.local_dim
            fuse_p = self.planes(f"{tag}fuse_l_p", f * (h // 8) * (w // 8), ld)
            src, outs = None, []
            for st in (1, 2, 3):
                hs, ws = h >> st, w >> st
                ap = self.planes(f"{tag}e{st}a_p", f * hs * ws, d[st])
                if st == 1:
                    ops.stem_fused(x0, P["stem"], ap)
                else:
                    self._conv_p(ops, P, f"feat_extracts.{st}.0", src, stride=2, sink=ap)
                if st == 3:
                    self._c3p(ops, P, "feat_extracts.3.1", ap, f, hs, ws, sink=fuse_p, sink_c0=ld - d[3])
                    outs.append(_PMap(fuse_p, f, hs, ws, 0, ld))
                else:
                    ep = self.planes(f"{tag}e{st}_p", f * hs * ws, d[st])
                    self._c3p(ops, P, f"feat_extracts.{st}.1", ap, f, hs, ws, sink=ep)
                    outs.append(_PMap(ep, f, hs, ws, 0, d[st]))
                    src = outs[-1]
            return outs[0], outs[1], outs[2]
        a = self.buf(f"{tag}e0a", f, h, w, d[0]); self._conv_act(ops, P, "feat_extracts.0.0", x0[..., :3], a)
        e0 = self.buf(f"{tag}e0", f, h, w, d[0]); self._conv_act(ops, P, "feat_extracts.0.1", a, e0)
        a = self.buf(f"{tag}e1a", f, h // 2, w // 2, d[1]); self._conv_act(ops, P, "feat_extracts.1.0", e0, a, 2)
        e1 = self.buf(f"{tag}e1", f, h // 2, w // 2, d[1]); self._conv_act(ops, P, "feat_extracts.1.1", a, e1)
        a = self.buf(f"{tag}e2a", f, h // 4, w // 4, d[2]); self._conv_act(ops, P, "feat_extracts.2.0", e1, a, 2)
        e2 = self.buf(f"{tag}e2", f, h // 4, w // 4, d[2]); self._conv_act(ops, P, "feat_extracts.2.1", a, e2)
        a = self.buf(f"{tag}e3a", f, h // 8, w // 8, d[3]); self._conv_act(ops, P, "feat_extracts.3.0", e2, a, 2)
        fuse = self.buf(f"{tag}fuse_l", f, h // 8, w // 8, self._v.local_dim)
        self._conv_act(ops, P, "feat_extracts.3.1", a, fuse[..., self._v.local_dim - d[3]:])
        return e1, e2, fuse

    def _fusion(self, ops, P, p, fine, mid, fuse, c_mid, c_fine, tag):
        if isinstance(fuse, _PMap):
            f, h, w, c = fuse.n, fuse.h, fuse.w, fuse.c
            self._conv_p(ops, P, f"{p}.layers.0", mid, stride=2, pad=1, dil=1, act=False, sink=fuse.p, sink_c0=0)
            self._conv_p(ops, P, f"{p}.layers.1", fine, stride=4, pad=1, dil=1, act=False, sink=fuse.p, sink_c0=c_mid)
            self._conv_p(ops, P, f"{p}.layers.2", fine, stride=4, pad=2, dil=2, act=False, sink=fuse.p, sink_c0=c_mid + c_fine)
            t = self.buf(f"{tag}fproj", f * h * w, c)
            ops.linear(fuse.p, P[f"pk:{p}.proj.weight"], t, bias=P[f"{p}.proj.bias"])
            out = self.buf(f"{tag}fnorm", f * h * w, c)
            ops.layernorm(t, out, P[f"{p}.norm.weight"], P[f"{p}.norm.bias"])
            return out
        f, h, w, c = fuse.shape
        self._conv_plain(ops, P, f"{p}.layers.0", mid, fuse[..., 0:c_mid], stride=2, pad=1, dil=1)
        self._conv_plain(ops, P, f"{p}.layers.1", fine, fuse[..., c_mid:c_mid + c_fine], stride=4, pad=1, dil=1)
        self._conv_plain(ops, P, f"{p}.layers.2", fine, fuse[..., c_mid + c_fine:c_mid + 2 * c_fine], stride=4, pad=2, dil=2)
        t = self.buf(f"{tag}fproj", f * h * w, c)
        ops.linear(fuse.reshape(f * h * w, c), P[f"pk:{p}.proj.weight"], t, bias=P[f"{p}.proj.bias"])
        out = self.buf(f"{tag}fnorm", f * h * w, c)
        ops.layernorm(t, out, P[f"{p}.norm.weight"], P[f"{p}.norm.bias"])
        return out

    @staticmethod
    def _stacked(buf, off, c):
        b, h, w, ld = buf.shape
        flat = buf.reshape(b * h * w, ld)[:, off:off + 2 * c]
        return flat.unflatten(1, (2, c)).permute(1, 0, 2)

    def _motion_branch(self, ops, P, branch, mlp, x_tokens, b, h, w, ws, tag):
        c = x_tokens.shape[-1]
        cin = 8 + 2 * c
        mlp_in = self.buf(f"{tag}mlp_in", b, h, w, cin)
        flat = mlp_in.reshape(b * h * w, cin)
        pc = self._plane_convs(ops)
        mlp_in_p = self.planes(f"{tag}mlp_in_p", b * h * w, cin) if pc else None
        x = x_tokens
        for blk in range(2):
            mdst = flat[:, 4 * blk:4 * blk + 4].unflatten(1, (2, 2)).permute(1, 0, 2)
            out = self._stacked(mlp_in, 8, c) if blk == 1 else self.buf(f"{tag}blk0", 2 * b * h * w, c)
            msink = (mlp_in_p, 4 * blk, 2) if (pc and getattr(ops, "motion_head_sink", False)) else None
            self._block(ops, P, f"{branch}.{blk}", x, 2 * b, h, w, ws, 0 if blk == 0 else ws // 2, True, out, mdst, tag,
                        out_sink=(mlp_in_p, 8, c) if (pc and blk == 1) else None, motion_sink=msink)
            x = out
        hid = P[f"{mlp}.0.0.bias"].shape[0]
        if pc:
            if not getattr(ops, "motion_head_sink", False):
                ops.split_planes(flat[:, 0:8], mlp_in_p, c0=0)
            t1p = self.planes(f"{tag}mm1_p", b * h * w, hid)
            t2p = self.planes(f"{tag}mm2_p", b * h * w, hid)
            self._c3p(ops, P, f"{mlp}.0", mlp_in_p, b, h, w, sink=t1p)
            self._c3p(ops, P, f"{mlp}.1", t1p, b, h, w, sink=t2p)
            return mlp_in, t2p
        t1 = self.buf(f"{tag}mm1", b, h, w, hid); self._conv_act(ops, P, f"{mlp}.0", mlp_in, t1)
        t2 = self.buf(f"{tag}mm2", b, h, w, hid); self._conv_act(ops, P, f"{mlp}.1", t1, t2)
        return mlp_in, t2

    def _global_tokens(self, ops, P, e2, fuse_l, tag):
        v = self._v
        d = v.hidden_dims
        if isinstance(fuse_l, _PMap):
            f, h8, w8 = fuse_l.n, fuse_l.h, fuse_l.w
            h_, w_ = h8 // 2, w8 // 2
            s3 = _PMap(fuse_l.p, f, h8, w8, (v.local_dim - d[3]) // 32, d[3])
            fuse_g = _PMap(self.planes(f"{tag}fuse_g_p", f * h_ * w_, v.global_dim), f, h_, w_, 0, v.global_dim)
            ap = self.planes(f"{tag}ga_p", f * h_ * w_, v.last_feat_dim)
            self._conv_p(ops, P, "last_feat_extract.0", s3, stride=2, sink=ap)
            self._c3p(ops, P, "last_feat_extract.1", ap, f, h_, w_, sink=fuse_g.p, sink_c0=d[3] + 2 * d[2])
            return self._fusion(ops, P, "global_feature_fusion", e2, s3, fuse_g, d[3], d[2], tag + "g")
        f, h8, w8, _ = fuse_l.shape
        h_, w_ = h8 // 2, w8 // 2
        s3 = fuse_l[..., v.local_dim - d[3]:]
        fuse_g = self.buf(f"{tag}fuse_g", f, h_, w_, v.global_dim)
        a = self.buf(f"{tag}ga", f, h_, w_, v.last_feat_dim)
        self._conv_act(ops, P, "last_feat_extract.0", s3, a, 2)
        self._conv_act(ops, P, "last_feat_extract.1", a, fuse_g[..., d[3] + 2 * d[2]:])
        return self._fusion(ops, P, "global_feature_fusion", e2, s3, fuse_g, d[3], d[2], tag + "g")

    def _global_from_tokens(self, ops, P, tokens, b, h_, w_, tag):
        mlp_in, t2 = self._motion_branch(ops, P, "global_motion_atmformer", "global_motion_mlp", tokens, b, h_, w_,
                                         self.global_motion_args["window_size"], tag + "g")
        gout = self.buf(f"{tag}gout", b, h_, w_, 8)
        self._head1x1(ops, P, "global_motion_mlp.2", t2, b, h_, w_, gout[..., :5])
        return gout

    def _global_motion(self, ops, P, e2, fuse_l, b, tag):
        if isinstance(fuse_l, _PMap):
            h_, w_ = fuse_l.h // 2, fuse_l.w // 2
        else:
            h_, w_ = fuse_l.shape[1] // 2, fuse_l.shape[2] // 2
        tokens = self._global_tokens(ops, P, e2, fuse_l, tag)
        return self._global_from_tokens(ops, P, tokens, b, h_, w_, tag)

    def _head1x1(self, ops, P, p, t2, b, h, w, out):
        if isinstance(t2, Planes):
            ops.head1x1_planes(t2, b, h, w, P[f"pk:{p}.weight"], out, bias=P[f"{p}.bias"])
        else:
            self._conv_plain(ops, P, p, t2, out, pad=0)

    def _ensemble_flows(self, ops, P, im0, im1):
        b, _, h, w = im0.shape
        cands, losses = [], []
        c0, c1 = im0, im1
        for lvl in range(3):
            if lvl:
# ... 654 lines not shown
```

### include/atmvfi.h

```cpp
#ifndef ATMVFI_H
#define ATMVFI_H

#include <stdint.h>

#ifdef __cplusplus
extern "C" {
#endif

#define ATMVFI_OK        0
#define ATMVFI_EINVAL   -1
#define ATMVFI_EALIGN   -2
#define ATMVFI_ELAUNCH  -3

int         atmvfi_version(void);
const char* atmvfi_last_error(void);
const char* atmvfi_source_digest(void);
int atmvfi_range_word_set(uint32_t* word, void* stream);
int atmvfi_range_checked(void);

#define ATMVFI_GEMM_CONV   0
#define ATMVFI_GEMM_LINEAR 1
#define ATMVFI_GEMM_DECONV 2

typedef struct atmvfi_gemm_params {
    int32_t mode;
    const float* in;
    int32_t in_ld, N, H, W, Cin;
    int64_t in_gstride; int32_t in_rpg;
    const float* weight;
    int32_t Cout, kh, kw, stride, pad, dil;
    int32_t Ho, Wo;
    int64_t M;
    float* out;
    int32_t out_ld;
    int64_t out_gstride; int32_t out_rpg;
    const int32_t* out_row_map;
    const float* bias;
    const float* prelu;
    const float* in_prelu;
    const float* residual;
    int32_t res_ld;
    int32_t precision;
    const void* weight_hi;
    const void* weight_lo;
    const void* in_hi;
    const void* in_lo;
    void* out_hi;
    void* out_lo;
    int64_t out_plane_rows;
    int32_t out_plane_c0, out_plane_gc;
    int32_t tile_wn;
    const void* in_hi2;
    const void* in_lo2;
    int32_t in_ld2, in_split_chunks;
    float* workspace;
    int64_t workspace_floats;
} atmvfi_gemm_params;

#define ATMVFI_PREC_F32   0
#define ATMVFI_PREC_F16X3 1

int atmvfi_gemm(const atmvfi_gemm_params* p, void* stream);
int64_t atmvfi_gemm_workspace_floats(int64_t M, int ngemm, int ksteps);

int atmvfi_head1x1_planes(const void* in_hi, const void* in_lo, int64_t plane_rows, int64_t rows, int Cin, const float* weight,
                          const float* bias, int Cout, float* out, int out_ld, void* stream);

int atmvfi_split_planes(const float* in, int in_ld, int64_t M, int C, const float* prelu, void* hi, void* lo, int plane_rows, void* stream);
int atmvfi_split_planes_at(const float* in, int in_ld, int64_t M, int C, const float* prelu, void* hi, void* lo, int plane_rows, int c0,
                           int pad_to, void* stream);

int atmvfi_conv2d(const atmvfi_gemm_params* p, void* stream);
int atmvfi_linear(const atmvfi_gemm_params* p, void* stream);
int atmvfi_deconv2x2(const atmvfi_gemm_params* p, void* stream);

int64_t atmvfi_packed_weight_floats(int mode, int Cout, int Cin, int kh, int kw);
int atmvfi_pack_weight(int mode, const float* src, float* dst, int Cout, int Cin, int kh, int kw, void* stream);

int64_t atmvfi_split_weight_halves(int mode, int Cout, int Cin, int kh, int kw);
int atmvfi_pack_weight_split(int mode, const float* src, void* dst_hi, void* dst_lo, int Cout, int Cin, int kh, int kw,
                             void* stream);
int64_t atmvfi_conv3x3_weight_halves(int Cout, int Cin);
int atmvfi_pack_weight_conv3x3(const float* src, void* dst_hi, void* dst_lo, int Cout, int Cin, void* stream);
int atmvfi_conv3x3_f16x3(const float* in, int in_ld, int N, int H, int W, int Cin, const void* w_hi, const void* w_lo,
                         int Cout, float* out, int out_ld, const float* bias, const float* prelu, void* out_hi, void* out_lo,
                         int64_t plane_rows, const float* plane_prelu, int schedule, int wn, void* stream);
int atmvfi_conv3x3_planes(const void* in_hi, const void* in_lo, int64_t in_rows, int N, int H, int W, int Cin, const void* w_hi,
                          const void* w_lo, int Cout, float* out, int out_ld, const float* bias, const float* prelu, void* out_hi,
                          void* out_lo, int64_t plane_rows, int out_c0, const float* plane_prelu, int out_cmin, int wn, void* stream);
int atmvfi_conv3x3_planes2(const void* in_hi, const void* in_lo, int64_t in_rows, int N, int H, int W, int Cin, const void* w_hi,
                           const void* w_lo, int Cout, float* out, int out_ld, const float* bias, const float* prelu, void* out_hi,
                           void* out_lo, int64_t plane_rows, int out_c0, const float* plane_prelu, void* out_hi2, void* out_lo2,
                           int64_t plane_rows2, int out_c02, int out_cmin, int wn, void* stream);
int64_t atmvfi_conv3x3_planes_workspace_floats(int N, int H, int W, int Cin, int Cout);
int atmvfi_conv3x3_planes3(const void* in_hi, const void* in_lo, int64_t in_rows, int N, int H, int W, int Cin, const void* w_hi,
                           const void* w_lo, int Cout, float* out, int out_ld, const float* bias, const float* prelu, void* out_hi,
                           void* out_lo, int64_t plane_rows, int out_c0, const float* plane_prelu, void* out_hi2, void* out_lo2,
                           int64_t plane_rows2, int out_c02, int out_cmin, int wn, float* workspace, int64_t workspace_floats, void* stream);
int atmvfi_layernorm(const float* in, int in_ld, int64_t in_gstride, int in_rpg,
                     const int32_t* src_row_map, float* out, int out_ld,
                     const float* gamma, const float* beta, int64_t rows, int C,
                     void* out_hi, void* out_lo, int plane_rows, void* stream);

int atmvfi_dwconv3x3_gelu(const float* in, int in_ld, float* out, int out_ld,
                          const float* weight9, const float* bias,
                          int N, int H, int W, int C, void* out_hi, void* out_lo, int plane_rows, void* stream);
int atmvfi_pack_dw_weight(const float* src , float* dst , int C, void* stream);

int atmvfi_window_attention(const float* qkv, float* out , float* motion,
                            const int32_t* labels, int Bw, int nW, int ws, int heads, int hd,
                            int kv_shift, void* out_hi, void* out_lo, int plane_rows, void* stream);
int atmvfi_window_attention_f16x3(const float* qkv, float* out , float* motion,
                                  const int32_t* labels, int Bw, int nW, int ws, int heads, int hd,
                                  int kv_shift, void* out_hi, void* out_lo, int plane_rows, void* stream);
int atmvfi_window_attn_cross_motion(const float* qkv, float* out, float* motion, const int32_t* labels,
                                    int Bw, int nW, int ws, int heads, int hd, void* stream);
int atmvfi_window_attn_self(const float* qkv, float* out, const int32_t* labels,
                            int Bw, int nW, int ws, int heads, int hd, void* stream);

int atmvfi_motion_head(const float* motion , const int32_t* row_map,
                       const float* w0 , const float* b0, const float* w1 ,
                       const float* b1, float* out, int out_ld, int64_t out_gstride, int out_rpg,
                       int64_t rows, int heads, void* stream);
int atmvfi_motion_head_planes(const float* motion, const int32_t* row_map, const float* w0, const float* b0, const float* w1,
                              const float* b1, float* out, int out_ld, int64_t out_gstride, int out_rpg, int64_t rows, int heads,
                              void* out_hi, void* out_lo, int64_t plane_rows, int plane_c0, int plane_gc, void* stream);

int atmvfi_flow_warp(const float* src , const float* flow, int64_t flow_bstride,
                     int flow_pstride, int flow_cstride, float* dst, int B, int C, int H, int W, void* stream);
int atmvfi_flow_warp_tiled(const float* src , const float* flow, int64_t flow_bstride,
                           int flow_pstride, int flow_cstride, float* dst, int B, int C, int H, int W, void* stream);
int atmvfi_flow_warp_ex(const float* src , const float* flow , float* dst, uint8_t* mask ,
                        int B, int C, int H, int W, int padding_mode, void* stream);
int atmvfi_flow_warp_nhwc(const float* src, int src_ld, int64_t src_bstride,
                          const float* flow, int64_t flow_bstride, int flow_pstride, int flow_cstride,
                          float* dst, int dst_ld, int64_t dst_bstride, int B, int C, int H, int W, void* stream);

int atmvfi_warp_blend(const float* im0, const float* im1 ,
                      const float* motion, int motion_ld, int64_t motion_bstride,
                      float* i0w, float* i1w, float* it ,
                      float* flow0_out, float* flow1_out , float* mask1_out, float* mask2_out ,
                      const float* orig0, const float* orig1, float* pack15, int pack_ld,
                      int B, int H, int W, void* stream);
int atmvfi_warp_blend_planes(const float* im0, const float* im1, const float* motion, int motion_ld, int64_t motion_bstride,
                             float* i0w, float* i1w, float* it, float* flow0_out, float* flow1_out, float* mask1_out, float* mask2_out,
                             const float* orig0, const float* orig1, float* pack15, int pack_ld, void* pack_hi, void* pack_lo,
                             int64_t pack_rows, int pack_c0, int B, int H, int W, void* stream);
int atmvfi_warp_blend_tiled(const float* im0, const float* im1, const float* motion, int motion_ld, int64_t motion_bstride,
                            float* i0w, float* i1w, float* it, float* flow0_out, float* flow1_out, float* mask1_out, float* mask2_out,
                            const float* orig0, const float* orig1, float* pack15, int pack_ld, void* pack_hi, void* pack_lo,
                            int64_t pack_rows, int pack_c0, int B, int H, int W, void* stream);
#define atmvfi_blend atmvfi_warp_blend

int atmvfi_resize_bilinear_ac(const float* src, int64_t src_bstride, int64_t src_cstride, int64_t src_ystride,
                              int64_t src_xstride, float* dst, int B, int C, int Hi, int Wi, int Ho, int Wo,
                              float value_scale, void* stream);

int atmvfi_image_pyramid(const float* im0, const float* im1, float* l1, float* l2, float* l3, int B, int H, int W, void* stream);
int atmvfi_image_pyramid_pack(const float* im0, const float* im1, float* l1, float* l2, float* l3, float* pack, int B, int H, int W,
                              void* stream);

int atmvfi_flow_warp_up2(const float* src, const float* flow, float* dst, float* flow_up, int B, int C, int H, int W, void* stream);
int atmvfi_flow_warp_up2_tiled(const float* src, const float* flow, float* dst, float* flow_up, int B, int C, int H, int W, void* stream);

int atmvfi_pack_frames(const float* im0, const float* im1, float* dst , int B, int H, int W, void* stream);

int atmvfi_final_residual(const float* it , const float* r, int r_ld,
                          float* it_sum, float* it_clamped, int B, int H, int W, void* stream);

int atmvfi_conv3x3_planes_readout(const void* in_hi, const void* in_lo, int64_t in_rows, int N, int H, int W, int Cin, const void* w_hi,
                                  const void* w_lo, int Cout, const float* bias, const float* prelu, const void* w2, float* contrib,
                                  int64_t contrib_plane, void* stream);
int atmvfi_refine_tail(const float* contrib, int64_t contrib_plane, const float* bias , const float* slope ,
                       const float* it , float* it_sum, float* it_clamped, int B, int H, int W, void* stream);

int atmvfi_frame_u8_to_f32(const void* src, int H, int W, int bgr, float* dst, int Hp, int Wp, int pad_top, int pad_left, void* stream);
int atmvfi_frame_f32_to_u8(const float* src, int Hp, int Wp, int pad_top, int pad_left, void* dst, int H, int W, int bgr, void* stream);
int atmvfi_frame_u8_window(const void* src, int H, int W, int bgr, int mode, int y0, int x0, int h, int w, float* dst, int Hp, int Wp,
                           int pad_top, int pad_left, void* dst_u8, void* stream);

int atmvfi_pool_blocks(void* pool, int64_t slot_bytes, int n_slots, const int32_t* slots , int n ,
                       int64_t block_bytes, void* buf, int to_pool, void* stream);
int atmvfi_tta_merge(const float* pred , const float* pred_flip , float* out ,
                     void* out_u8 , int Hp, int Wp, int pad_top, int pad_left, int H, int W, int bgr, void* stream);
int atmvfi_frame_rot180(const float* src , float* dst, int C, int Hp, int Wp, void* stream);

int64_t atmvfi_frame_signature_workspace_ints(int h, int w);
int atmvfi_frame_signature(const void* src, int H, int W, int bgr, int y0, int x0, int h, int w, int32_t* sig , int32_t* workspace,
                           int64_t workspace_ints, void* stream);

int64_t atmvfi_frame_difference_workspace_ints(int h, int w);
int atmvfi_frame_difference(const void* a, const void* b, int H, int W, int bgr, int y0, int x0, int h, int w, int32_t* out ,
                            int32_t* workspace, int64_t workspace_ints, void* stream);

int64_t atmvfi_frame_borders_workspace_ints(int H, int W);
int atmvfi_frame_borders(const void* src, int H, int W, int bgr, int32_t* out , int32_t* workspace, int64_t workspace_ints,
                         void* stream);
int atmvfi_frame_compose(void* dst , const void* border , int H, int W, int y0, int x0, int h, int w,
                         const float* src , int Hp, int Wp, int pad_top, int pad_left,
                         const void* win_u8 , int bgr, void* stream);

int atmvfi_shutter_accumulate(int32_t* acc , int h, int w, const float* src, int Hp, int Wp, int pad_top, int pad_left,
                              const uint8_t* src_u8 , int bgr, int weight, int light, int first, void* stream);
int atmvfi_shutter_resolve(const int32_t* acc, int h, int w, int total_weight, int light, uint8_t* dst_u8 , int bgr, void* stream);
int atmvfi_shutter_table(int light, uint16_t out[256]);

int atmvfi_yuv420_to_rgb(const void* yuv, int H, int W, int depth, int matrix, int full_range, int siting, void* dst_u8, int bgr,
                         float* dst, int Hp, int Wp, int pad_top, int pad_left, void* stream);
int atmvfi_rgb_to_yuv420(const void* src_u8, int bgr, const float* src, int Hp, int Wp, int pad_top, int pad_left, int H, int W,
                         int matrix, int full_range, int siting, void* yuv, void* stream);

int atmvfi_yuv420_window(const void* yuv, int H, int W, int depth, int matrix, int full_range, int siting, int mode, int y0, int x0, int h,
                         int w, float* dst, int Hp, int Wp, int pad_top, int pad_left, void* dst_u8, void* stream);

int atmvfi_yuv420p10_to_f32(const void* yuv, int H, int W, int matrix, int siting, int y0, int x0, int h, int w, float* dst, int Hp, int Wp,
                            int pad_top, int pad_left, void* stream);
int atmvfi_f32_to_yuv420p10(const float* src, int Hp, int Wp, int pad_top, int pad_left, int H, int W, int matrix, int siting, void* yuv,
                            void* stream);

int atmvfi_yuv_surface_decode(const void* yuv, int H, int W, int depth, int matrix, int full_range, int siting, int chroma, int msb,
                              int64_t pitch, int64_t chroma_pitch, int64_t chroma_offset, int keep_depth, int y0, int x0, int h, int w,
                              void* dst_u8, int bgr, float* dst, int Hp, int Wp, int pad_top, int pad_left, void* stream);
int atmvfi_yuv_surface_encode(const void* src_u8, int bgr, const float* src, int Hp, int Wp, int pad_top, int pad_left, int H, int W,
                              int depth, int matrix, int full_range, int siting, int chroma, int msb, void* yuv, void* stream);

int atmvfi_yuv_sub_decode(const void* yuv, int H, int W, int depth, int matrix, int full_range, int siting, int subsampling, int chroma, int msb,
                          int64_t pitch, int64_t chroma_pitch, int64_t chroma_offset, int keep_depth, int y0, int x0, int h, int w,
                          void* dst_u8, int bgr, float* dst, int Hp, int Wp, int pad_top, int pad_left, void* stream);
int atmvfi_yuv_sub_encode(const void* src_u8, int bgr, const float* src, int Hp, int Wp, int pad_top, int pad_left, int H, int W,
                          int depth, int matrix, int full_range, int siting, int subsampling, int chroma, int msb, void* yuv, void* stream);

int64_t atmvfi_l1_mean_workspace_floats(int B, int64_t per_sample);
int atmvfi_l1_mean(const float* a, const float* b, float* out, int B, int64_t per_sample, float* workspace, int64_t workspace_floats, void* stream);
int atmvfi_ensemble_select(const float* loss0, const float* loss1, const float* loss2, const float* c0_l0, const float* c1_l0,
                           const float* c0_l1, const float* c1_l1, const float* c0_l2, const float* c1_l2, float* out0, float* out1, int B,
                           int64_t per_sample, void* stream);

int atmvfi_stem_fused(const float* x, int F, int H, int W, int C0, int C1, const void* w1_hi, const void* w1_lo, const float* b1, const float* p1,
                      const void* w2_hi, const void* w2_lo, const float* b2, const float* p2, const void* w3_hi, const void* w3_lo,
                      const float* b3, const float* p3, void* out_hi, void* out_lo, int64_t out_plane_rows, void* stream);

#define ATMVFI_SSIM_X_U8 1
#define ATMVFI_SSIM_X_BGR 2
#define ATMVFI_SSIM_ROUND_Y 4
#define ATMVFI_SSIM_ACCUMULATE 8
#define ATMVFI_SSIM_MSE_F32 16
#define ATMVFI_SSIM_FLAG_MASK 31
int64_t atmvfi_ssim_psnr_workspace_floats(int B, int H, int W);
int atmvfi_ssim_psnr(const void* x, int64_t x_bstride, int64_t x_cstride, int64_t x_ystride, int64_t x_xstride, const float* y,
                     int64_t y_bstride, int64_t y_cstride, int64_t y_ystride, int64_t y_xstride, int B, int H, int W, float val_range,
                     int flags, double* out, float* workspace, int64_t workspace_floats, void* stream);
// ... 18 lines not shown
```

Measured before the change: 51.42.

## Add dedicated stride-2 3x3 conv kernel on fp16 planes with warp-specialized loaders

```diff
diff --git a/atm-vfi_amd/csrc/api.hip b/atm-vfi_amd/csrc/api.hip
--- a/atm-vfi_amd/csrc/api.hip
+++ b/atm-vfi_amd/csrc/api.hip
@@ -55,7 +55,7 @@
 #endif
 }
 
-extern "C" int atmvfi_version(void) { return (0 << 16) | (21 << 8) | 0; }
+extern "C" int atmvfi_version(void) { return (0 << 16) | (22 << 8) | 0; }
 extern "C" const char* atmvfi_last_error(void) { return atmvfi::g_err; }
 #ifndef ATMVFI_SOURCE_DIGEST
 #define ATMVFI_SOURCE_DIGEST "unknown (api.hip compiled outside the Makefile)"
diff --git a/atm-vfi_amd/csrc/conv3x3s2_planes.hip b/atm-vfi_amd/csrc/conv3x3s2_planes.hip
--- /dev/null
+++ b/atm-vfi_amd/csrc/conv3x3s2_planes.hip
@@ -0,0 +1,283 @@
+#include "conv3_common.h"
+
+namespace {
+
+constexpr int S2_TH = 8, S2_TW = 16;
+constexpr int S2_HH = 2 * S2_TH + 1, S2_HWD = 2 * S2_TW + 1;
+constexpr int S2_EVEN = S2_TW + 1;
+constexpr int S2_PIX = S2_HH * S2_HWD;
+constexpr int S2_PIECES = (S2_PIX + 15) / 16;
+constexpr int S2_PLANE = S2_PIECES * 1024;
+constexpr int S2_BUF = 2 * S2_PLANE;
+constexpr int S2_LOADERS = 4;
+constexpr int S2_LPIECES = S2_PIECES / S2_LOADERS;
+static_assert(S2_PIECES % S2_LOADERS == 0, "whole pieces per loader");
+constexpr int S2_THREADS = (8 + S2_LOADERS) * 64;
+
+struct S2Dev {
+    const unsigned char* in_hi;
+    const unsigned char* in_lo;
+    const unsigned char* in_hi2;
+    const unsigned char* in_lo2;
+    long long chunk_bytes, chunk_bytes2;
+    int split, nchunks;
+    int N, H, W, Ho, Wo;
+    const unsigned char* w_hi;
+    const unsigned char* w_lo;
+    int wrows;
+    int Cout;
+    float* out;
+    int out_ld;
+    const float* bias;
+    const float* prelu;
+    _Float16* out_hi;
+    _Float16* out_lo;
+    long long plane_rows;
+    int out_c0;
+    int tiles_x, tiles_y, nblocks, ntiles, vblocks;
+};
+
+template <int WNW>
+__global__ __launch_bounds__(S2_THREADS) void conv3x3s2_planes_kernel(const S2Dev a) {
+    fp16_saturate_on();
+    constexpr int BN = 64 * WNW;
+    extern __shared__ __attribute__((aligned(16))) unsigned char smem[];
+    const int tid = threadIdx.x;
+    const int lane = tid & 63;
+    const int wave = __builtin_amdgcn_readfirstlane(tid >> 6);
+    const int grid = gridDim.x;
+
+    auto decode = [&](int v, int& img, int& oy0, int& ox0, int& n0) -> bool {
+        const int slot = v >> 3;
+        const int sgrp = slot / a.nblocks;
+        const int L = sgrp * 8 + (v & 7);
+        if (v >= a.vblocks || L >= a.ntiles) return false;
+        const int per_img = a.tiles_x * a.tiles_y;
+        img = L / per_img;
+        const int rem = L - img * per_img;
+        const int ty = rem / a.tiles_x;
+        oy0 = ty * S2_TH;
+        ox0 = (rem - ty * a.tiles_x) * S2_TW;
+        n0 = (slot - sgrp * a.nblocks) * BN;
+        return true;
+    };
+    int v = blockIdx.x;
+    int img, oy0, ox0, n0;
+    if (!decode(v, img, oy0, ox0, n0)) return;
+
+    if (wave >= 8) {
+        const int lw = wave - 8;
+        unsigned hoff[S2_LPIECES];
+        const long long zero_row = (long long)a.N * a.H * a.W;
+        auto setup = [&]() {
+#pragma unroll
+            for (int k = 0; k < S2_LPIECES; ++k) {
+                const int s = lw + S2_LOADERS * k;
+                const int p = 16 * s + (lane >> 2);
+                const int hy = p / S2_HWD, q = p - hy * S2_HWD;
+                const int hx = q < S2_EVEN ? 2 * q : 2 * (q - S2_EVEN) + 1;
+                const int iy = 2 * oy0 - 1 + hy, ix = 2 * ox0 - 1 + hx;
+                const bool ok = p < S2_PIX && (unsigned)iy < (unsigned)a.H && (unsigned)ix < (unsigned)a.W;
+                const long long row = ok ? ((long long)img * a.H + iy) * a.W + ix : zero_row;
+                hoff[k] = (unsigned)(row * 64 + (((lane & 3) ^ swz64(p)) << 4));
+            }
+        };
+        auto issue = [&](int c, int buf) {
+            const bool second = c >= a.split;
+            const unsigned char* bh = second ? a.in_hi2 + (long long)(c - a.split) * a.chunk_bytes2 : a.in_hi + (long long)c * a.chunk_bytes;
+            const unsigned char* bl = second ? a.in_lo2 + (long long)(c - a.split) * a.chunk_bytes2 : a.in_lo + (long long)c * a.chunk_bytes;
+            unsigned char* dst = smem + buf * S2_BUF + lw * 1024;
+#pragma unroll
+            for (int k = 0; k < S2_LPIECES; ++k) {
+                const int s = S2_LOADERS * k;
+                __builtin_amdgcn_global_load_lds((const __attribute__((address_space(1))) void*)(bh + hoff[k]),
+                                                 (__attribute__((address_space(3))) void*)(dst + s * 1024), 16, 0, 0);
+                __builtin_amdgcn_global_load_lds((const __attribute__((address_space(1))) void*)(bl + hoff[k]),
+                                                 (__attribute__((address_space(3))) void*)(dst + S2_PLANE + s * 1024), 16, 0, 0);
+            }
+        };
+        setup();
+        issue(0, 0);
+        asm volatile("s_waitcnt vmcnt(0)" ::: "memory");
+        __syncthreads();
+        int buf = 0, c = 0;
+        for (;;) {
+            bool more = true;
+            if (++c == a.nchunks) {
+                c = 0;
+                v += grid;
+                more = decode(v, img, oy0, ox0, n0);
+                if (more) setup();
+            }
+            buf ^= 1;
+            if (more) issue(c, buf);
+            asm volatile("s_waitcnt vmcnt(0)" ::: "memory");
+            __syncthreads();
+            if (!more) break;
+        }
+        return;
+    }
+
+    const int r = lane & 15, g = lane >> 4;
+    const int wr = wave & 1, wc = wave >> 1;
+    const int prow = 8 * wr * S2_HWD + r;
+    unsigned xa[8];
+#pragma unroll
+    for (int k = 0; k < 8; ++k) xa[k] = (unsigned)(prow * 64 + ((g ^ swz64(prow + k)) << 4));
+    const unsigned step_bytes = (unsigned)a.wrows * 64u;
+    const unsigned tap_bytes = (unsigned)a.nchunks * step_bytes;
+    const auto rs_hi = __builtin_amdgcn_make_buffer_rsrc(const_cast<unsigned char*>(a.w_hi), 0, 9 * tap_bytes, 0x00020000);
+    const auto rs_lo = __builtin_amdgcn_make_buffer_rsrc(const_cast<unsigned char*>(a.w_lo), 0, 9 * tap_bytes, 0x00020000);
+
+    for (int buf = 0;;) {
+        unsigned woff[WNW];
+#pragma unroll
+        for (int j = 0; j < WNW; ++j) {
+            const int rg = n0 + (wc * WNW + j) * 16;
+            woff[j] = (unsigned)(((rg < a.wrows ? rg : 0) + r) * 64 + g * 16);
+        }
+        f32x4 acc[4][WNW], cor[4][WNW];
+#pragma unroll
+        for (int i = 0; i < 4; ++i)
+#pragma unroll
+            for (int j = 0; j < WNW; ++j) acc[i][j] = cor[i][j] = (f32x4){0.f, 0.f, 0.f, 0.f};
+
+        f16x8 wh[3][WNW], wl[3][WNW];
+        auto load_w = [&](auto setc, unsigned kbytes) {
+            constexpr int SET = decltype(setc)::value;
+#pragma unroll
+            for (int j = 0; j < WNW; ++j) {
+                wh[SET][j] = __builtin_bit_cast(f16x8, __builtin_amdgcn_raw_buffer_load_b128(rs_hi, woff[j], kbytes, 0));
+                wl[SET][j] = __builtin_bit_cast(f16x8, __builtin_amdgcn_raw_buffer_load_b128(rs_lo, woff[j], kbytes, 0));
+            }
+        };
+        load_w(std::integral_constant<int, 0>{}, 0u);
+        load_w(std::integral_constant<int, 1>{}, tap_bytes);
+        for (int c = 0; c < a.nchunks; ++c) {
+            __syncthreads();
+            const unsigned char* hb = smem + buf * S2_BUF;
+            const unsigned this_c = (unsigned)c * step_bytes;
+            const unsigned next_c = (unsigned)(c + 1 < a.nchunks ? c + 1 : 0) * step_bytes;
+            static_for<0, 9>([&](auto tc) {
+                constexpr int T = decltype(tc)::value;
+                constexpr int KY = T / 3, KX = T % 3;
+                constexpr int KOFF = KX == 0 ? 0 : KX == 1 ? S2_EVEN : 1;
+                constexpr int SET = T % 3;
+                load_w(std::integral_constant<int, (T + 2) % 3>{}, T + 2 < 9 ? this_c + (T + 2) * tap_bytes : next_c + (T + 2 - 9) * tap_bytes);
+                __builtin_amdgcn_sched_barrier(0);
+                f16x8 xh[4], xl[4];
+#pragma unroll
+                for (int i = 0; i < 4; ++i) {
+                    const int C = (2 * i + KY) * S2_HWD + KOFF;
+                    xh[i] = *reinterpret_cast<const f16x8*>(hb + xa[C & 7] + 64 * C);
+                    xl[i] = *reinterpret_cast<const f16x8*>(hb + xa[C & 7] + 64 * C + S2_PLANE);
+                }
+#pragma unroll
+                for (int j = 0; j < WNW; ++j) {
+#pragma unroll
+                    for (int i = 0; i < 4; ++i) cor[i][j] = __builtin_amdgcn_mfma_f32_16x16x32_f16(wl[SET][j], xh[i], cor[i][j], 0, 0, 0);
+#pragma unroll
+                    for (int i = 0; i < 4; ++i) acc[i][j] = __builtin_amdgcn_mfma_f32_16x16x32_f16(wh[SET][j], xh[i], acc[i][j], 0, 0, 0);
+#pragma unroll
+                    for (int i = 0; i < 4; ++i) cor[i][j] = __builtin_amdgcn_mfma_f32_16x16x32_f16(wh[SET][j], xl[i], cor[i][j], 0, 0, 0);
+                }
+                __builtin_amdgcn_sched_barrier(0);
+            });
+            buf ^= 1;
+        }
+
+#pragma unroll
+        for (int j = 0; j < WNW; ++j) {
+            const int co = n0 + (wc * WNW + j) * 16 + 4 * g;
+            const bool col_ok = co < a.Cout;
+            const f32x4 bv = (a.bias && col_ok) ? *reinterpret_cast<const f32x4*>(a.bias + co) : (f32x4){0.f, 0.f, 0.f, 0.f};
+            const f32x4 sl = (a.prelu && col_ok) ? *reinterpret_cast<const f32x4*>(a.prelu + co) : (f32x4){1.f, 1.f, 1.f, 1.f};
+#pragma unroll
+            for (int i = 0; i < 4; ++i) {
+                const int oy = oy0 + 4 * wr + i, ox = ox0 + r;
+                if (!(col_ok && oy < a.Ho && ox < a.Wo)) continue;
+                f32x4 o = acc[i][j] + cor[i][j] * LO_UNSCALE + bv;
+                if (a.prelu) o = (f32x4){o.x > 0.f ? o.x : sl.x * o.x, o.y > 0.f ? o.y : sl.y * o.y, o.z > 0.f ? o.z : sl.z * o.z, o.w > 0.f ? o.w : sl.w * o.w};
+                const long long row = ((long long)img * a.Ho + oy) * a.Wo + ox;
+                if (a.out) *reinterpret_cast<f32x4*>(a.out + row * a.out_ld + co) = o;
+                if (a.out_hi) sink_store4(RowSink{nullptr, 0, a.out_hi, a.out_lo, a.plane_rows}, row, a.out_c0 + co, o);
+            }
+        }
+        v += grid;
+        if (!decode(v, img, oy0, ox0, n0)) break;
+    }
+    __syncthreads();
+}
+
+template <int WNW>
+int launch_s2(const S2Dev& d, hipStream_t s) {
+    constexpr size_t lds = 2 * S2_BUF;
+    static_assert(lds <= 160 * 1024, "LDS budget");
+    const hipError_t attr_err = atmvfi::allow_dynamic_lds<conv3x3s2_planes_kernel<WNW>>(lds);
+    ATMVFI_REQUIRE(attr_err == hipSuccess, ATMVFI_ELAUNCH, "conv3x3s2_planes: hipFuncSetAttribute: %s", hipGetErrorString(attr_err));
+    S2Dev ds = d;
+    ds.nblocks = (d.Cout + 64 * WNW - 1) / (64 * WNW);
+    const long long vblocks = ((long long)d.ntiles + 7) / 8 * 8 * ds.nblocks;
+    ATMVFI_REQUIRE(vblocks < (1ll << 31), ATMVFI_EINVAL, "conv3x3s2_planes: grid too large");
+    ds.vblocks = (int)vblocks;
+    const int grid = std::min(ds.vblocks, atmvfi::cu_count());
+    hipLaunchKernelGGL(conv3x3s2_planes_kernel<WNW>, dim3((unsigned)grid), dim3(S2_THREADS), lds, s, ds);
+    return atmvfi::check_launch("conv3x3s2_planes");
+}
+
+}
+
+extern "C" int atmvfi_conv3x3s2_planes_routed(int N, int H, int W, int Cin, int Cout) {
+    if (N <= 0 || H <= 0 || W <= 0 || Cin <= 0 || Cout <= 0 || Cout % 4 != 0) return 0;
+    const long long tiles = (long long)N * (((H - 1) / 2 + 1 + S2_TH - 1) / S2_TH) * (((W - 1) / 2 + 1 + S2_TW - 1) / S2_TW);
+    return Cout <= 128 && Cin % 32 == 0 && tiles >= atmvfi::cu_count();
+}
+
+extern "C" int atmvfi_conv3x3s2_planes(const void* in_hi, const void* in_lo, int64_t in_rows, const void* in_hi2, const void* in_lo2,
+                                       int64_t in_rows2, int split_chunks, int N, int H, int W, int Cin, const void* w_hi, const void* w_lo,
+                                       int Cout, float* out, int out_ld, const float* bias, const float* prelu, void* out_hi, void* out_lo,
+                                       int64_t plane_rows, int out_c0, void* stream) {
+    ATMVFI_REQUIRE(in_hi && in_lo && w_hi && w_lo && (out || out_hi), ATMVFI_EINVAL, "conv3x3s2_planes: null pointer");
+    ATMVFI_REQUIRE(N > 0 && H > 0 && W > 0 && Cin > 0 && Cout > 0 && Cout % 4 == 0, ATMVFI_EINVAL,
+                   "conv3x3s2_planes: bad shape (Cout must be a multiple of 4, got %d)", Cout);
+    const int nchunks = (Cin + 31) / 32;
+    const int64_t rows = (int64_t)N * H * W;
+    ATMVFI_REQUIRE(in_rows > rows && in_rows * 64 < (1ll << 32), ATMVFI_EINVAL,
+                   "conv3x3s2_planes: in_rows %lld must exceed N*H*W (the zero row) and in_rows * 64 must fit 32 bits", (long long)in_rows);
+    ATMVFI_REQUIRE((in_hi2 == nullptr) == (in_lo2 == nullptr), ATMVFI_EINVAL, "conv3x3s2_planes: the second source needs both planes");
+    if (in_hi2)
+        ATMVFI_REQUIRE(split_chunks > 0 && split_chunks < nchunks && in_rows2 > rows && in_rows2 * 64 < (1ll << 32), ATMVFI_EINVAL,
+                       "conv3x3s2_planes: the second source needs 0 < split_chunks < chunks, in_rows2 > N*H*W and in_rows2 * 64 within 32 bits");
+    ATMVFI_REQUIRE(atmvfi::aligned16(in_hi) && atmvfi::aligned16(in_lo) && atmvfi::aligned16(in_hi2) && atmvfi::aligned16(in_lo2) &&
+                       atmvfi::aligned16(w_hi) && atmvfi::aligned16(w_lo) && atmvfi::aligned16(bias) && atmvfi::aligned16(prelu),
+                   ATMVFI_EALIGN, "conv3x3s2_planes: pointers (incl. bias/prelu) must be 16-byte aligned");
+    const int Ho = (H - 1) / 2 + 1, Wo = (W - 1) / 2 + 1;
+    if (out)
+        ATMVFI_REQUIRE(atmvfi::aligned16(out) && out_ld % 4 == 0 && out_ld >= Cout, ATMVFI_EALIGN,
+                       "conv3x3s2_planes: fp32 output must be 16-byte aligned with ld %% 4 == 0 covering Cout");
+    ATMVFI_REQUIRE((out_hi == nullptr) == (out_lo == nullptr), ATMVFI_EINVAL, "conv3x3s2_planes: plane sink needs both planes");
+    if (out_hi) {
+        ATMVFI_REQUIRE(plane_rows >= (int64_t)N * Ho * Wo && out_c0 >= 0 && out_c0 % 4 == 0, ATMVFI_EINVAL,
+                       "conv3x3s2_planes: plane sink needs plane_rows >= N*Ho*Wo and a channel offset that is a multiple of 4");
+        ATMVFI_REQUIRE(atmvfi::aligned16(out_hi) && atmvfi::aligned16(out_lo), ATMVFI_EALIGN,
+                       "conv3x3s2_planes: plane sink pointers must be 16-byte aligned");
+    }
+    S2Dev d;
+    d.in_hi = (const unsigned char*)in_hi; d.in_lo = (const unsigned char*)in_lo;
+    d.in_hi2 = (const unsigned char*)in_hi2; d.in_lo2 = (const unsigned char*)in_lo2;
+    d.chunk_bytes = in_rows * 64; d.chunk_bytes2 = in_rows2 * 64;
+    d.split = in_hi2 ? split_chunks : nchunks; d.nchunks = nchunks;
+    d.N = N; d.H = H; d.W = W; d.Ho = Ho; d.Wo = Wo;
+    d.w_hi = (const unsigned char*)w_hi; d.w_lo = (const unsigned char*)w_lo;
+    d.wrows = atmvfi::round_up(Cout, 16);
+    ATMVFI_REQUIRE(9ll * nchunks * d.wrows * 64 < (1ll << 31), ATMVFI_EINVAL, "conv3x3s2_planes: a weight plane must stay below 2 GiB");
+    d.Cout = Cout; d.out = out; d.out_ld = out_ld; d.bias = bias; d.prelu = prelu;
+    d.out_hi = (_Float16*)out_hi; d.out_lo = (_Float16*)out_lo; d.plane_rows = plane_rows; d.out_c0 = out_c0;
+    d.tiles_x = (Wo + S2_TW - 1) / S2_TW; d.tiles_y = (Ho + S2_TH - 1) / S2_TH;
+    const long long ntiles = (long long)N * d.tiles_x * d.tiles_y;
+    ATMVFI_REQUIRE(ntiles < (1ll << 28), ATMVFI_EINVAL, "conv3x3s2_planes: too many tiles");
+    d.ntiles = (int)ntiles; d.nblocks = 0; d.vblocks = 0;
+    hipStream_t s = (hipStream_t)stream;
+    if (Cout <= 64) return launch_s2<1>(d, s);
+    return launch_s2<2>(d, s);
+}
diff --git a/atm-vfi_amd/csrc/plan_dispatch.inc b/atm-vfi_amd/csrc/plan_dispatch.inc
--- a/atm-vfi_amd/csrc/plan_dispatch.inc
+++ b/atm-vfi_amd/csrc/plan_dispatch.inc
@@ -1,4 +1,4 @@
-#define ATMVFI_PLAN_NFN 65
+#define ATMVFI_PLAN_NFN 66
 static const char* const kPlanFnNames[ATMVFI_PLAN_NFN] = {
     "atmvfi_conv2d",
     "atmvfi_conv3x3_f16x3",
@@ -6,6 +6,7 @@
     "atmvfi_conv3x3_planes2",
     "atmvfi_conv3x3_planes3",
     "atmvfi_conv3x3_planes_readout",
+    "atmvfi_conv3x3s2_planes",
     "atmvfi_deconv2x2",
     "atmvfi_dwconv3x3_gelu",
     "atmvfi_ensemble_select",
@@ -66,7 +67,7 @@
     "atmvfi_yuv_surface_decode",
     "atmvfi_yuv_surface_encode",
 };
-static const int kPlanFnArgs[ATMVFI_PLAN_NFN] = {1, 19, 21, 25, 27, 15, 1, 13, 13, 10, 8, 10, 9, 14, 10, 8, 8, 7, 15, 12, 9, 5, 11, 9, 15, 1, 10, 8, 9, 7, 14, 1, 12, 17, 3, 6, 7, 5, 8, 8, 1, 10, 13, 13, 13, 7, 8, 10, 18, 21, 11, 19, 23, 23, 13, 13, 9, 8, 14, 18, 14, 25, 17, 24, 16};
+static const int kPlanFnArgs[ATMVFI_PLAN_NFN] = {1, 19, 21, 25, 27, 15, 22, 1, 13, 13, 10, 8, 10, 9, 14, 10, 8, 8, 7, 15, 12, 9, 5, 11, 9, 15, 1, 10, 8, 9, 7, 14, 1, 12, 17, 3, 6, 7, 5, 8, 8, 1, 10, 13, 13, 13, 7, 8, 10, 18, 21, 11, 19, 23, 23, 13, 13, 9, 8, 14, 18, 14, 25, 17, 24, 16};
 static int plan_call(const atmvfi_plan_op* op, void* stream) {
     const atmvfi_plan_arg* a = op->a;
     switch (op->fn) {
@@ -76,65 +77,66 @@
     case 3: return atmvfi_conv3x3_planes2((const void*)(uintptr_t)a[0].u, (const void*)(uintptr_t)a[1].u, (int64_t)a[2].i, (int)a[3].i, (int)a[4].i, (int)a[5].i, (int)a[6].i, (const void*)(uintptr_t)a[7].u, (const void*)(uintptr_t)a[8].u, (int)a[9].i, (float*)(uintptr_t)a[10].u, (int)a[11].i, (const float*)(uintptr_t)a[12].u, (const float*)(uintptr_t)a[13].u, (void*)(uintptr_t)a[14].u, (void*)(uintptr_t)a[15].u, (int64_t)a[16].i, (int)a[17].i, (const float*)(uintptr_t)a[18].u, (void*)(uintptr_t)a[19].u, (void*)(uintptr_t)a[20].u, (int64_t)a[21].i, (int)a[22].i, (int)a[23].i, (int)a[24].i, stream);
     case 4: return atmvfi_conv3x3_planes3((const void*)(uintptr_t)a[0].u, (const void*)(uintptr_t)a[1].u, (int64_t)a[2].i, (int)a[3].i, (int)a[4].i, (int)a[5].i, (int)a[6].i, (const void*)(uintptr_t)a[7].u, (const void*)(uintptr_t)a[8].u, (int)a[9].i, (float*)(uintptr_t)a[10].u, (int)a[11].i, (const float*)(uintptr_t)a[12].u, (const float*)(uintptr_t)a[13].u, (void*)(uintptr_t)a[14].u, (void*)(uintptr_t)a[15].u, (int64_t)a[16].i, (int)a[17].i, (const float*)(uintptr_t)a[18].u, (void*)(uintptr_t)a[19].u, (void*)(uintptr_t)a[20].u, (int64_t)a[21].i, (int)a[22].i, (int)a[23].i, (int)a[24].i, (float*)(uintptr_t)a[25].u, (int64_t)a[26].i, stream);
     case 5: return atmvfi_conv3x3_planes_readout((const void*)(uintptr_t)a[0].u, (const void*)(uintptr_t)a[1].u, (int64_t)a[2].i, (int)a[3].i, (int)a[4].i, (int)a[5].i, (int)a[6].i, (const void*)(uintptr_t)a[7].u, (const void*)(uintptr_t)a[8].u, (int)a[9].i, (const float*)(uintptr_t)a[10].u, (const float*)(uintptr_t)a[11].u, (const void*)(uintptr_t)a[12].u, (float*)(uintptr_t)a[13].u, (int64_t)a[14].i, stream);
-    case 6: return atmvfi_deconv2x2((const atmvfi_gemm_params*)(uintptr_t)a[0].u, stream);
-    case 7: return atmvfi_dwconv3x3_gelu((const float*)(uintptr_t)a[0].u, (int)a[1].i, (float*)(uintptr_t)a[2].u, (int)a[3].i, (const float*)(uintptr_t)a[4].u, (const float*)(uintptr_t)a[5].u, (int)a[6].i, (int)a[7].i, (int)a[8].i, (int)a[9].i, (void*)(uintptr_t)a[10].u, (void*)(uintptr_t)a[11].u, (int)a[12].i, stream);
-    case 8: return atmvfi_ensemble_select((const float*)(uintptr_t)a[0].u, (const float*)(uintptr_t)a[1].u, (const float*)(uintptr_t)a[2].u, (const float*)(uintptr_t)a[3].u, (const float*)(uintptr_t)a[4].u, (const float*)(uintptr_t)a[5].u, (const float*)(uintptr_t)a[6].u, (const float*)(uintptr_t)a[7].u, (const float*)(uintptr_t)a[8].u, (float*)(uintptr_t)a[9].u, (float*)(uintptr_t)a[10].u, (int)a[11].i, (int64_t)a[12].i, stream);
-    case 9: return atmvfi_f32_to_yuv420p10((const float*)(uintptr_t)a[0].u, (int)a[1].i, (int)a[2].i, (int)a[3].i, (int)a[4].i, (int)a[5].i, (int)a[6].i, (int)a[7].i, (int)a[8].i, (void*)(uintptr_t)a[9].u, stream);
-    case 10: return atmvfi_final_residual((const float*)(uintptr_t)a[0].u, (const float*)(uintptr_t)a[1].u, (int)a[2].i, (float*)(uintptr_t)a[3].u, (float*)(uintptr_t)a[4].u, (int)a[5].i, (int)a[6].i, (int)a[7].i, stream);
-    case 11: return atmvfi_flow_warp((const float*)(uintptr_t)a[0].u, (const float*)(uintptr_t)a[1].u, (int64_t)a[2].i, (int)a[3].i, (int)a[4].i, (float*)(uintptr_t)a[5].u, (int)a[6].i, (int)a[7].i, (int)a[8].i, (int)a[9].i, stream);
-    case 12: return atmvfi_flow_warp_ex((const float*)(uintptr_t)a[0].u, (const float*)(uintptr_t)a[1].u, (float*)(uintptr_t)a[2].u, (uint8_t*)(uintptr_t)a[3].u, (int)a[4].i, (int)a[5].i, (int)a[6].i, (int)a[7].i, (int)a[8].i, stream);
-    case 13: return atmvfi_flow_warp_nhwc((const float*)(uintptr_t)a[0].u, (int)a[1].i, (int64_t)a[2].i, (const float*)(uintptr_t)a[3].u, (int64_t)a[4].i, (int)a[5].i, (int)a[6].i, (float*)(uintptr_t)a[7].u, (int)a[8].i, (int64_t)a[9].i, (int)a[10].i, (int)a[11].i, (int)a[12].i, (int)a[13].i, stream);
-    case 14: return atmvfi_flow_warp_tiled((const float*)(uintptr_t)a[0].u, (const float*)(uintptr_t)a[1].u, (int64_t)a[2].i, (int)a[3].i, (int)a[4].i, (float*)(uintptr_t)a[5].u, (int)a[6].i, (int)a[7].i, (int)a[8].i, (int)a[9].i, stream);
-    case 15: return atmvfi_flow_warp_up2((const float*)(uintptr_t)a[0].u, (const float*)(uintptr_t)a[1].u, (float*)(uintptr_t)a[2].u, (float*)(uintptr_t)a[3].u, (int)a[4].i, (int)a[5].i, (int)a[6].i, (int)a[7].i, stream);
-    case 16: return atmvfi_flow_warp_up2_tiled((const float*)(uintptr_t)a[0].u, (const float*)(uintptr_t)a[1].u, (float*)(uintptr_t)a[2].u, (float*)(uintptr_t)a[3].u, (int)a[4].i, (int)a[5].i, (int)a[6].i, (int)a[7].i, stream);
-    case 17: return atmvfi_frame_borders((const void*)(uintptr_t)a[0].u, (int)a[1].i, (int)a[2].i, (int)a[3].i, (int32_t*)(uintptr_t)a[4].u, (int32_t*)(uintptr_t)a[5].u, (int64_t)a[6].i, stream);
-    case 18: return atmvfi_frame_compose((void*)(uintptr_t)a[0].u, (const void*)(uintptr_t)a[1].u, (int)a[2].i, (int)a[3].i, (int)a[4].i, (int)a[5].i, (int)a[6].i, (int)a[7].i, (const float*)(uintptr_t)a[8].u, (int)a[9].i, (int)a[10].i, (int)a[11].i, (int)a[12].i, (const void*)(uintptr_t)a[13].u, (int)a[14].i, stream);
-    case 19: return atmvfi_frame_difference((const void*)(uintptr_t)a[0].u, (const void*)(uintptr_t)a[1].u, (int)a[2].i, (int)a[3].i, (int)a[4].i, (int)a[5].i, (int)a[6].i, (int)a[7].i, (int)a[8].i, (int32_t*)(uintptr_t)a[9].u, (int32_t*)(uintptr_t)a[10].u, (int64_t)a[11].i, stream);
-    case 20: return atmvfi_frame_f32_to_u8((const float*)(uintptr_t)a[0].u, (int)a[1].i, (int)a[2].i, (int)a[3].i, (int)a[4].i, (void*)(uintptr_t)a[5].u, (int)a[6].i, (int)a[7].i, (int)a[8].i, stream);
-    case 21: return atmvfi_frame_rot180((const float*)(uintptr_t)a[0].u, (float*)(uintptr_t)a[1].u, (int)a[2].i, (int)a[3].i, (int)a[4].i, stream);
-    case 22: return atmvfi_frame_signature((const void*)(uintptr_t)a[0].u, (int)a[1].i, (int)a[2].i, (int)a[3].i, (int)a[4].i, (int)a[5].i, (int)a[6].i, (int)a[7].i, (int32_t*)(uintptr_t)a[8].u, (int32_t*)(uintptr_t)a[9].u, (int64_t)a[10].i, stream);
-    case 23: return atmvfi_frame_u8_to_f32((const void*)(uintptr_t)a[0].u, (int)a[1].i, (int)a[2].i, (int)a[3].i, (float*)(uintptr_t)a[4].u, (int)a[5].i, (int)a[6].i, (int)a[7].i, (int)a[8].i, stream);
-    case 24: return atmvfi_frame_u8_window((const void*)(uintptr_t)a[0].u, (int)a[1].i, (int)a[2].i, (int)a[3].i, (int)a[4].i, (int)a[5].i, (int)a[6].i, (int)a[7].i, (int)a[8].i, (float*)(uintptr_t)a[9].u, (int)a[10].i, (int)a[11].i, (int)a[12].i, (int)a[13].i, (void*)(uintptr_t)a[14].u, stream);
-    case 25: return atmvfi_gemm((const atmvfi_gemm_params*)(uintptr_t)a[0].u, stream);
-    case 26: return atmvfi_head1x1_planes((const void*)(uintptr_t)a[0].u, (const void*)(uintptr_t)a[1].u, (int64_t)a[2].i, (int64_t)a[3].i, (int)a[4].i, (const float*)(uintptr_t)a[5].u, (const float*)(uintptr_t)a[6].u, (int)a[7].i, (float*)(uintptr_t)a[8].u, (int)a[9].i, stream);
-    case 27: return atmvfi_image_pyramid((const float*)(uintptr_t)a[0].u, (const float*)(uintptr_t)a[1].u, (float*)(uintptr_t)a[2].u, (float*)(uintptr_t)a[3].u, (float*)(uintptr_t)a[4].u, (int)a[5].i, (int)a[6].i, (int)a[7].i, stream);
-    case 28: return atmvfi_image_pyramid_pack((const float*)(uintptr_t)a[0].u, (const float*)(uintptr_t)a[1].u, (float*)(uintptr_t)a[2].u, (float*)(uintptr_t)a[3].u, (float*)(uintptr_t)a[4].u, (float*)(uintptr_t)a[5].u, (int)a[6].i, (int)a[7].i, (int)a[8].i, stream);
-    case 29: return atmvfi_l1_mean((const float*)(uintptr_t)a[0].u, (const float*)(uintptr_t)a[1].u, (float*)(uintptr_t)a[2].u, (int)a[3].i, (int64_t)a[4].i, (float*)(uintptr_t)a[5].u, (int64_t)a[6].i, stream);
-    case 30: return atmvfi_layernorm((const float*)(uintptr_t)a[0].u, (int)a[1].i, (int64_t)a[2].i, (int)a[3].i, (const int32_t*)(uintptr_t)a[4].u, (float*)(uintptr_t)a[5].u, (int)a[6].i, (const float*)(uintptr_t)a[7].u, (const float*)(uintptr_t)a[8].u, (int64_t)a[9].i, (int)a[10].i, (void*)(uintptr_t)a[11].u, (void*)(uintptr_t)a[12].u, (int)a[13].i, stream);
-    case 31: return atmvfi_linear((const atmvfi_gemm_params*)(uintptr_t)a[0].u, stream);
-    case 32: return atmvfi_motion_head((const float*)(uintptr_t)a[0].u, (const int32_t*)(uintptr_t)a[1].u, (const float*)(uintptr_t)a[2].u, (const float*)(uintptr_t)a[3].u, (const float*)(uintptr_t)a[4].u, (const float*)(uintptr_t)a[5].u, (float*)(uintptr_t)a[6].u, (int)a[7].i, (int64_t)a[8].i, (int)a[9].i, (int64_t)a[10].i, (int)a[11].i, stream);
-    case 33: return atmvfi_motion_head_planes((const float*)(uintptr_t)a[0].u, (const int32_t*)(uintptr_t)a[1].u, (const float*)(uintptr_t)a[2].u, (const float*)(uintptr_t)a[3].u, (const float*)(uintptr_t)a[4].u, (const float*)(uintptr_t)a[5].u, (float*)(uintptr_t)a[6].u, (int)a[7].i, (int64_t)a[8].i, (int)a[9].i, (int64_t)a[10].i, (int)a[11].i, (void*)(uintptr_t)a[12].u, (void*)(uintptr_t)a[13].u, (int64_t)a[14].i, (int)a[15].i, (int)a[16].i, stream);
-    case 34: return atmvfi_pack_dw_weight((const float*)(uintptr_t)a[0].u, (float*)(uintptr_t)a[1].u, (int)a[2].i, stream);
-    case 35: return atmvfi_pack_frames((const float*)(uintptr_t)a[0].u, (const float*)(uintptr_t)a[1].u, (float*)(uintptr_t)a[2].u, (int)a[3].i, (int)a[4].i, (int)a[5].i, stream);
-    case 36: return atmvfi_pack_weight((int)a[0].i, (const float*)(uintptr_t)a[1].u, (float*)(uintptr_t)a[2].u, (int)a[3].i, (int)a[4].i, (int)a[5].i, (int)a[6].i, stream);
-    case 37: return atmvfi_pack_weight_conv3x3((const float*)(uintptr_t)a[0].u, (void*)(uintptr_t)a[1].u, (void*)(uintptr_t)a[2].u, (int)a[3].i, (int)a[4].i, stream);
-    case 38: return atmvfi_pack_weight_split((int)a[0].i, (const float*)(uintptr_t)a[1].u, (void*)(uintptr_t)a[2].u, (void*)(uintptr_t)a[3].u, (int)a[4].i, (int)a[5].i, (int)a[6].i, (int)a[7].i, stream);
-    case 39: return atmvfi_pool_blocks((void*)(uintptr_t)a[0].u, (int64_t)a[1].i, (int)a[2].i, (const int32_t*)(uintptr_t)a[3].u, (int)a[4].i, (int64_t)a[5].i, (void*)(uintptr_t)a[6].u, (int)a[7].i, stream);
-    case 40: return atmvfi_range_word_set((uint32_t*)(uintptr_t)a[0].u, stream);
-    case 41: return atmvfi_refine_tail((const float*)(uintptr_t)a[0].u, (int64_t)a[1].i, (const float*)(uintptr_t)a[2].u, (const float*)(uintptr_t)a[3].u, (const float*)(uintptr_t)a[4].u, (float*)(uintptr_t)a[5].u, (float*)(uintptr_t)a[6].u, (int)a[7].i, (int)a[8].i, (int)a[9].i, stream);
-    case 42: return atmvfi_resize_bilinear_ac((const float*)(uintptr_t)a[0].u, (int64_t)a[1].i, (int64_t)a[2].i, (int64_t)a[3].i, (int64_t)a[4].i, (float*)(uintptr_t)a[5].u, (int)a[6].i, (int)a[7].i, (int)a[8].i, (int)a[9].i, (int)a[10].i, (int)a[11].i, (float)a[12].f, stream);
-    case 43: return atmvfi_rgb_to_yuv420((const void*)(uintptr_t)a[0].u, (int)a[1].i, (const float*)(uintptr_t)a[2].u, (int)a[3].i, (int)a[4].i, (int)a[5].i, (int)a[6].i, (int)a[7].i, (int)a[8].i, (int)a[9].i, (int)a[10].i, (int)a[11].i, (void*)(uintptr_t)a[12].u, stream);
-    case 44: return atmvfi_shutter_accumulate((int32_t*)(uintptr_t)a[0].u, (int)a[1].i, (int)a[2].i, (const float*)(uintptr_t)a[3].u, (int)a[4].i, (int)a[5].i, (int)a[6].i, (int)a[7].i, (const uint8_t*)(uintptr_t)a[8].u, (int)a[9].i, (int)a[10].i, (int)a[11].i, (int)a[12].i, stream);
-    case 45: return atmvfi_shutter_resolve((const int32_t*)(uintptr_t)a[0].u, (int)a[1].i, (int)a[2].i, (int)a[3].i, (int)a[4].i, (uint8_t*)(uintptr_t)a[5].u, (int)a[6].i, stream);
-    case 46: return atmvfi_split_planes((const float*)(uintptr_t)a[0].u, (int)a[1].i, (int64_t)a[2].i, (int)a[3].i, (const float*)(uintptr_t)a[4].u, (void*)(uintptr_t)a[5].u, (void*)(uintptr_t)a[6].u, (int)a[7].i, stream);
-    case 47: return atmvfi_split_planes_at((const float*)(uintptr_t)a[0].u, (int)a[1].i, (int64_t)a[2].i, (int)a[3].i, (const float*)(uintptr_t)a[4].u, (void*)(uintptr_t)a[5].u, (void*)(uintptr_t)a[6].u, (int)a[7].i, (int)a[8].i, (int)a[9].i, stream);
-    case 48: return atmvfi_ssim_psnr((const void*)(uintptr_t)a[0].u, (int64_t)a[1].i, (int64_t)a[2].i, (int64_t)a[3].i, (int64_t)a[4].i, (const float*)(uintptr_t)a[5].u, (int64_t)a[6].i, (int64_t)a[7].i, (int64_t)a[8].i, (int64_t)a[9].i, (int)a[10].i, (int)a[11].i, (int)a[12].i, (float)a[13].f, (int)a[14].i, (double*)(uintptr_t)a[15].u, (float*)(uintptr_t)a[16].u, (int64_t)a[17].i, stream);
-    case 49: return atmvfi_stem_fused((const float*)(uintptr_t)a[0].u, (int)a[1].i, (int)a[2].i, (int)a[3].i, (int)a[4].i, (int)a[5].i, (const void*)(uintptr_t)a[6].u, (const void*)(uintptr_t)a[7].u, (const float*)(uintptr_t)a[8].u, (const float*)(uintptr_t)a[9].u, (const void*)(uintptr_t)a[10].u, (const void*)(uintptr_t)a[11].u, (const float*)(uintptr_t)a[12].u, (const float*)(uintptr_t)a[13].u, (const void*)(uintptr_t)a[14].u, (const void*)(uintptr_t)a[15].u, (const float*)(uintptr_t)a[16].u, (const float*)(uintptr_t)a[17].u, (void*)(uintptr_t)a[18].u, (void*)(uintptr_t)a[19].u, (int64_t)a[20].i, stream);
-    case 50: return atmvfi_tta_merge((const float*)(uintptr_t)a[0].u, (const float*)(uintptr_t)a[1].u, (float*)(uintptr_t)a[2].u, (void*)(uintptr_t)a[3].u, (int)a[4].i, (int)a[5].i, (int)a[6].i, (int)a[7].i, (int)a[8].i, (int)a[9].i, (int)a[10].i, stream);
-    case 51: return atmvfi_warp_blend((const float*)(uintptr_t)a[0].u, (const float*)(uintptr_t)a[1].u, (const float*)(uintptr_t)a[2].u, (int)a[3].i, (int64_t)a[4].i, (float*)(uintptr_t)a[5].u, (float*)(uintptr_t)a[6].u, (float*)(uintptr_t)a[7].u, (float*)(uintptr_t)a[8].u, (float*)(uintptr_t)a[9].u, (float*)(uintptr_t)a[10].u, (float*)(uintptr_t)a[11].u, (const float*)(uintptr_t)a[12].u, (const float*)(uintptr_t)a[13].u, (float*)(uintptr_t)a[14].u, (int)a[15].i, (int)a[16].i, (int)a[17].i, (int)a[18].i, stream);
-    case 52: return atmvfi_warp_blend_planes((const float*)(uintptr_t)a[0].u, (const float*)(uintptr_t)a[1].u, (const float*)(uintptr_t)a[2].u, (int)a[3].i, (int64_t)a[4].i, (float*)(uintptr_t)a[5].u, (float*)(uintptr_t)a[6].u, (float*)(uintptr_t)a[7].u, (float*)(uintptr_t)a[8].u, (float*)(uintptr_t)a[9].u, (float*)(uintptr_t)a[10].u, (float*)(uintptr_t)a[11].u, (const float*)(uintptr_t)a[12].u, (const float*)(uintptr_t)a[13].u, (float*)(uintptr_t)a[14].u, (int)a[15].i, (void*)(uintptr_t)a[16].u, (void*)(uintptr_t)a[17].u, (int64_t)a[18].i, (int)a[19].i, (int)a[20].i, (int)a[21].i, (int)a[22].i, stream);
-    case 53: return atmvfi_warp_blend_tiled((const float*)(uintptr_t)a[0].u, (const float*)(uintptr_t)a[1].u, (const float*)(uintptr_t)a[2].u, (int)a[3].i, (int64_t)a[4].i, (float*)(uintptr_t)a[5].u, (float*)(uintptr_t)a[6].u, (float*)(uintptr_t)a[7].u, (float*)(uintptr_t)a[8].u, (float*)(uintptr_t)a[9].u, (float*)(uintptr_t)a[10].u, (float*)(uintptr_t)a[11].u, (const float*)(uintptr_t)a[12].u, (const float*)(uintptr_t)a[13].u, (float*)(uintptr_t)a[14].u, (int)a[15].i, (void*)(uintptr_t)a[16].u, (void*)(uintptr_t)a[17].u, (int64_t)a[18].i, (int)a[19].i, (int)a[20].i, (int)a[21].i, (int)a[22].i, stream);
-    case 54: return atmvfi_window_attention((const float*)(uintptr_t)a[0].u, (float*)(uintptr_t)a[1].u, (float*)(uintptr_t)a[2].u, (const int32_t*)(uintptr_t)a[3].u, (int)a[4].i, (int)a[5].i, (int)a[6].i, (int)a[7].i, (int)a[8].i, (int)a[9].i, (void*)(uintptr_t)a[10].u, (void*)(uintptr_t)a[11].u, (int)a[12].i, stream);
-    case 55: return atmvfi_window_attention_f16x3((const float*)(uintptr_t)a[0].u, (float*)(uintptr_t)a[1].u, (float*)(uintptr_t)a[2].u, (const int32_t*)(uintptr_t)a[3].u, (int)a[4].i, (int)a[5].i, (int)a[6].i, (int)a[7].i, (int)a[8].i, (int)a[9].i, (void*)(uintptr_t)a[10].u, (void*)(uintptr_t)a[11].u, (int)a[12].i, stream);
-    case 56: return atmvfi_window_attn_cross_motion((const float*)(uintptr_t)a[0].u, (float*)(uintptr_t)a[1].u, (float*)(uintptr_t)a[2].u, (const int32_t*)(uintptr_t)a[3].u, (int)a[4].i, (int)a[5].i, (int)a[6].i, (int)a[7].i, (int)a[8].i, stream);
-    case 57: return atmvfi_window_attn_self((const float*)(uintptr_t)a[0].u, (float*)(uintptr_t)a[1].u, (const int32_t*)(uintptr_t)a[2].u, (int)a[3].i, (int)a[4].i, (int)a[5].i, (int)a[6].i, (int)a[7].i, stream);
-    case 58: return atmvfi_yuv420_to_rgb((const void*)(uintptr_t)a[0].u, (int)a[1].i, (int)a[2].i, (int)a[3].i, (int)a[4].i, (int)a[5].i, (int)a[6].i, (void*)(uintptr_t)a[7].u, (int)a[8].i, (float*)(uintptr_t)a[9].u, (int)a[10].i, (int)a[11].i, (int)a[12].i, (int)a[13].i, stream);
-    case 59: return atmvfi_yuv420_window((const void*)(uintptr_t)a[0].u, (int)a[1].i, (int)a[2].i, (int)a[3].i, (int)a[4].i, (int)a[5].i, (int)a[6].i, (int)a[7].i, (int)a[8].i, (int)a[9].i, (int)a[10].i, (int)a[11].i, (float*)(uintptr_t)a[12].u, (int)a[13].i, (int)a[14].i, (int)a[15].i, (int)a[16].i, (void*)(uintptr_t)a[17].u, stream);
-    case 60: return atmvfi_yuv420p10_to_f32((const void*)(uintptr_t)a[0].u, (int)a[1].i, (int)a[2].i, (int)a[3].i, (int)a[4].i, (int)a[5].i, (int)a[6].i, (int)a[7].i, (int)a[8].i, (float*)(uintptr_t)a[9].u, (int)a[10].i, (int)a[11].i, (int)a[12].i, (int)a[13].i, stream);
-    case 61: return atmvfi_yuv_sub_decode((const void*)(uintptr_t)a[0].u, (int)a[1].i, (int)a[2].i, (int)a[3].i, (int)a[4].i, (int)a[5].i, (int)a[6].i, (int)a[7].i, (int)a[8].i, (int)a[9].i, (int64_t)a[10].i, (int64_t)a[11].i, (int64_t)a[12].i, (int)a[13].i, (int)a[14].i, (int)a[15].i, (int)a[16].i, (int)a[17].i, (void*)(uintptr_t)a[18].u, (int)a[19].i, (float*)(uintptr_t)a[20].u, (int)a[21].i, (int)a[22].i, (int)a[23].i, (int)a[24].i, stream);
-    case 62: return atmvfi_yuv_sub_encode((const void*)(uintptr_t)a[0].u, (int)a[1].i, (const float*)(uintptr_t)a[2].u, (int)a[3].i, (int)a[4].i, (int)a[5].i, (int)a[6].i, (int)a[7].i, (int)a[8].i, (int)a[9].i, (int)a[10].i, (int)a[11].i, (int)a[12].i, (int)a[13].i, (int)a[14].i, (int)a[15].i, (void*)(uintptr_t)a[16].u, stream);
-    case 63: return atmvfi_yuv_surface_decode((const void*)(uintptr_t)a[0].u, (int)a[1].i, (int)a[2].i, (int)a[3].i, (int)a[4].i, (int)a[5].i, (int)a[6].i, (int)a[7].i, (int)a[8].i, (int64_t)a[9].i, (int64_t)a[10].i, (int64_t)a[11].i, (int)a[12].i, (int)a[13].i, (int)a[14].i, (int)a[15].i, (int)a[16].i, (void*)(uintptr_t)a[17].u, (int)a[18].i, (float*)(uintptr_t)a[19].u, (int)a[20].i, (int)a[21].i, (int)a[22].i, (int)a[23].i, stream);
-    case 64: return atmvfi_yuv_surface_encode((const void*)(uintptr_t)a[0].u, (int)a[1].i, (const float*)(uintptr_t)a[2].u, (int)a[3].i, (int)a[4].i, (int)a[5].i, (int)a[6].i, (int)a[7].i, (int)a[8].i, (int)a[9].i, (int)a[10].i, (int)a[11].i, (int)a[12].i, (int)a[13].i, (int)a[14].i, (void*)(uintptr_t)a[15].u, stream);
+    case 6: return atmvfi_conv3x3s2_planes((const void*)(uintptr_t)a[0].u, (const void*)(uintptr_t)a[1].u, (int64_t)a[2].i, (const void*)(uintptr_t)a[3].u, (const void*)(uintptr_t)a[4].u, (int64_t)a[5].i, (int)a[6].i, (int)a[7].i, (int)a[8].i, (int)a[9].i, (int)a[10].i, (const void*)(uintptr_t)a[11].u, (const void*)(uintptr_t)a[12].u, (int)a[13].i, (float*)(uintptr_t)a[14].u, (int)a[15].i, (const float*)(uintptr_t)a[16].u, (const float*)(uintptr_t)a[17].u, (void*)(uintptr_t)a[18].u, (void*)(uintptr_t)a[19].u, (int64_t)a[20].i, (int)a[21].i, stream);
+    case 7: return atmvfi_deconv2x2((const atmvfi_gemm_params*)(uintptr_t)a[0].u, stream);
+    case 8: return atmvfi_dwconv3x3_gelu((const float*)(uintptr_t)a[0].u, (int)a[1].i, (float*)(uintptr_t)a[2].u, (int)a[3].i, (const float*)(uintptr_t)a[4].u, (const float*)(uintptr_t)a[5].u, (int)a[6].i, (int)a[7].i, (int)a[8].i, (int)a[9].i, (void*)(uintptr_t)a[10].u, (void*)(uintptr_t)a[11].u, (int)a[12].i, stream);
+    case 9: return atmvfi_ensemble_select((const float*)(uintptr_t)a[0].u, (const float*)(uintptr_t)a[1].u, (const float*)(uintptr_t)a[2].u, (const float*)(uintptr_t)a[3].u, (const float*)(uintptr_t)a[4].u, (const float*)(uintptr_t)a[5].u, (const float*)(uintptr_t)a[6].u, (const float*)(uintptr_t)a[7].u, (const float*)(uintptr_t)a[8].u, (float*)(uintptr_t)a[9].u, (float*)(uintptr_t)a[10].u, (int)a[11].i, (int64_t)a[12].i, stream);
+    case 10: return atmvfi_f32_to_yuv420p10((const float*)(uintptr_t)a[0].u, (int)a[1].i, (int)a[2].i, (int)a[3].i, (int)a[4].i, (int)a[5].i, (int)a[6].i, (int)a[7].i, (int)a[8].i, (void*)(uintptr_t)a[9].u, stream);
+    case 11: return atmvfi_final_residual((const float*)(uintptr_t)a[0].u, (const float*)(uintptr_t)a[1].u, (int)a[2].i, (float*)(uintptr_t)a[3].u, (float*)(uintptr_t)a[4].u, (int)a[5].i, (int)a[6].i, (int)a[7].i, stream);
+    case 12: return atmvfi_flow_warp((const float*)(uintptr_t)a[0].u, (const float*)(uintptr_t)a[1].u, (int64_t)a[2].i, (int)a[3].i, (int)a[4].i, (float*)(uintptr_t)a[5].u, (int)a[6].i, (int)a[7].i, (int)a[8].i, (int)a[9].i, stream);
+    case 13: return atmvfi_flow_warp_ex((const float*)(uintptr_t)a[0].u, (const float*)(uintptr_t)a[1].u, (float*)(uintptr_t)a[2].u, (uint8_t*)(uintptr_t)a[3].u, (int)a[4].i, (int)a[5].i, (int)a[6].i, (int)a[7].i, (int)a[8].i, stream);
+    case 14: return atmvfi_flow_warp_nhwc((const float*)(uintptr_t)a[0].u, (int)a[1].i, (int64_t)a[2].i, (const float*)(uintptr_t)a[3].u, (int64_t)a[4].i, (int)a[5].i, (int)a[6].i, (float*)(uintptr_t)a[7].u, (int)a[8].i, (int64_t)a[9].i, (int)a[10].i, (int)a[11].i, (int)a[12].i, (int)a[13].i, stream);
+    case 15: return atmvfi_flow_warp_tiled((const float*)(uintptr_t)a[0].u, (const float*)(uintptr_t)a[1].u, (int64_t)a[2].i, (int)a[3].i, (int)a[4].i, (float*)(uintptr_t)a[5].u, (int)a[6].i, (int)a[7].i, (int)a[8].i, (int)a[9].i, stream);
+    case 16: return atmvfi_flow_warp_up2((const float*)(uintptr_t)a[0].u, (const float*)(uintptr_t)a[1].u, (float*)(uintptr_t)a[2].u, (float*)(uintptr_t)a[3].u, (int)a[4].i, (int)a[5].i, (int)a[6].i, (int)a[7].i, stream);
+    case 17: return atmvfi_flow_warp_up2_tiled((const float*)(uintptr_t)a[0].u, (const float*)(uintptr_t)a[1].u, (float*)(uintptr_t)a[2].u, (float*)(uintptr_t)a[3].u, (int)a[4].i, (int)a[5].i, (int)a[6].i, (int)a[7].i, stream);
+    case 18: return atmvfi_frame_borders((const void*)(uintptr_t)a[0].u, (int)a[1].i, (int)a[2].i, (int)a[3].i, (int32_t*)(uintptr_t)a[4].u, (int32_t*)(uintptr_t)a[5].u, (int64_t)a[6].i, stream);
+    case 19: return atmvfi_frame_compose((void*)(uintptr_t)a[0].u, (const void*)(uintptr_t)a[1].u, (int)a[2].i, (int)a[3].i, (int)a[4].i, (int)a[5].i, (int)a[6].i, (int)a[7].i, (const float*)(uintptr_t)a[8].u, (int)a[9].i, (int)a[10].i, (int)a[11].i, (int)a[12].i, (const void*)(uintptr_t)a[13].u, (int)a[14].i, stream);
+    case 20: return atmvfi_frame_difference((const void*)(uintptr_t)a[0].u, (const void*)(uintptr_t)a[1].u, (int)a[2].i, (int)a[3].i, (int)a[4].i, (int)a[5].i, (int)a[6].i, (int)a[7].i, (int)a[8].i, (int32_t*)(uintptr_t)a[9].u, (int32_t*)(uintptr_t)a[10].u, (int64_t)a[11].i, stream);
+    case 21: return atmvfi_frame_f32_to_u8((const float*)(uintptr_t)a[0].u, (int)a[1].i, (int)a[2].i, (int)a[3].i, (int)a[4].i, (void*)(uintptr_t)a[5].u, (int)a[6].i, (int)a[7].i, (int)a[8].i, stream);
+    case 22: return atmvfi_frame_rot180((const float*)(uintptr_t)a[0].u, (float*)(uintptr_t)a[1].u, (int)a[2].i, (int)a[3].i, (int)a[4].i, stream);
+    case 23: return atmvfi_frame_signature((const void*)(uintptr_t)a[0].u, (int)a[1].i, (int)a[2].i, (int)a[3].i, (int)a[4].i, (int)a[5].i, (int)a[6].i, (int)a[7].i, (int32_t*)(uintptr_t)a[8].u, (int32_t*)(uintptr_t)a[9].u, (int64_t)a[10].i, stream);
+    case 24: return atmvfi_frame_u8_to_f32((const void*)(uintptr_t)a[0].u, (int)a[1].i, (int)a[2].i, (int)a[3].i, (float*)(uintptr_t)a[4].u, (int)a[5].i, (int)a[6].i, (int)a[7].i, (int)a[8].i, stream);
+    case 25: return atmvfi_frame_u8_window((const void*)(uintptr_t)a[0].u, (int)a[1].i, (int)a[2].i, (int)a[3].i, (int)a[4].i, (int)a[5].i, (int)a[6].i, (int)a[7].i, (int)a[8].i, (float*)(uintptr_t)a[9].u, (int)a[10].i, (int)a[11].i, (int)a[12].i, (int)a[13].i, (void*)(uintptr_t)a[14].u, stream);
+    case 26: return atmvfi_gemm((const atmvfi_gemm_params*)(uintptr_t)a[0].u, stream);
+    case 27: return atmvfi_head1x1_planes((const void*)(uintptr_t)a[0].u, (const void*)(uintptr_t)a[1].u, (int64_t)a[2].i, (int64_t)a[3].i, (int)a[4].i, (const float*)(uintptr_t)a[5].u, (const float*)(uintptr_t)a[6].u, (int)a[7].i, (float*)(uintptr_t)a[8].u, (int)a[9].i, stream);
+    case 28: return atmvfi_image_pyramid((const float*)(uintptr_t)a[0].u, (const float*)(uintptr_t)a[1].u, (float*)(uintptr_t)a[2].u, (float*)(uintptr_t)a[3].u, (float*)(uintptr_t)a[4].u, (int)a[5].i, (int)a[6].i, (int)a[7].i, stream);
+    case 29: return atmvfi_image_pyramid_pack((const float*)(uintptr_t)a[0].u, (const float*)(uintptr_t)a[1].u, (float*)(uintptr_t)a[2].u, (float*)(uintptr_t)a[3].u, (float*)(uintptr_t)a[4].u, (float*)(uintptr_t)a[5].u, (int)a[6].i, (int)a[7].i, (int)a[8].i, stream);
+    case 30: return atmvfi_l1_mean((const float*)(uintptr_t)a[0].u, (const float*)(uintptr_t)a[1].u, (float*)(uintptr_t)a[2].u, (int)a[3].i, (int64_t)a[4].i, (float*)(uintptr_t)a[5].u, (int64_t)a[6].i, stream);
+    case 31: return atmvfi_layernorm((const float*)(uintptr_t)a[0].u, (int)a[1].i, (int64_t)a[2].i, (int)a[3].i, (const int32_t*)(uintptr_t)a[4].u, (float*)(uintptr_t)a[5].u, (int)a[6].i, (const float*)(uintptr_t)a[7].u, (const float*)(uintptr_t)a[8].u, (int64_t)a[9].i, (int)a[10].i, (void*)(uintptr_t)a[11].u, (void*)(uintptr_t)a[12].u, (int)a[13].i, stream);
+    case 32: return atmvfi_linear((const atmvfi_gemm_params*)(uintptr_t)a[0].u, stream);
+    case 33: return atmvfi_motion_head((const float*)(uintptr_t)a[0].u, (const int32_t*)(uintptr_t)a[1].u, (const float*)(uintptr_t)a[2].u, (const float*)(uintptr_t)a[3].u, (const float*)(uintptr_t)a[4].u, (const float*)(uintptr_t)a[5].u, (float*)(uintptr_t)a[6].u, (int)a[7].i, (int64_t)a[8].i, (int)a[9].i, (int64_t)a[10].i, (int)a[11].i, stream);
+    case 34: return atmvfi_motion_head_planes((const float*)(uintptr_t)a[0].u, (const int32_t*)(uintptr_t)a[1].u, (const float*)(uintptr_t)a[2].u, (const float*)(uintptr_t)a[3].u, (const float*)(uintptr_t)a[4].u, (const float*)(uintptr_t)a[5].u, (float*)(uintptr_t)a[6].u, (int)a[7].i, (int64_t)a[8].i, (int)a[9].i, (int64_t)a[10].i, (int)a[11].i, (void*)(uintptr_t)a[12].u, (void*)(uintptr_t)a[13].u, (int64_t)a[14].i, (int)a[15].i, (int)a[16].i, stream);
+    case 35: return atmvfi_pack_dw_weight((const float*)(uintptr_t)a[0].u, (float*)(uintptr_t)a[1].u, (int)a[2].i, stream);
+    case 36: return atmvfi_pack_frames((const float*)(uintptr_t)a[0].u, (const float*)(uintptr_t)a[1].u, (float*)(uintptr_t)a[2].u, (int)a[3].i, (int)a[4].i, (int)a[5].i, stream);
+    case 37: return atmvfi_pack_weight((int)a[0].i, (const float*)(uintptr_t)a[1].u, (float*)(uintptr_t)a[2].u, (int)a[3].i, (int)a[4].i, (int)a[5].i, (int)a[6].i, stream);
+    case 38: return atmvfi_pack_weight_conv3x3((const float*)(uintptr_t)a[0].u, (void*)(uintptr_t)a[1].u, (void*)(uintptr_t)a[2].u, (int)a[3].i, (int)a[4].i, stream);
+    case 39: return atmvfi_pack_weight_split((int)a[0].i, (const float*)(uintptr_t)a[1].u, (void*)(uintptr_t)a[2].u, (void*)(uintptr_t)a[3].u, (int)a[4].i, (int)a[5].i, (int)a[6].i, (int)a[7].i, stream);
+    case 40: return atmvfi_pool_blocks((void*)(uintptr_t)a[0].u, (int64_t)a[1].i, (int)a[2].i, (const int32_t*)(uintptr_t)a[3].u, (int)a[4].i, (int64_t)a[5].i, (void*)(uintptr_t)a[6].u, (int)a[7].i, stream);
+    case 41: return atmvfi_range_word_set((uint32_t*)(uintptr_t)a[0].u, stream);
+    case 42: return atmvfi_refine_tail((const float*)(uintptr_t)a[0].u, (int64_t)a[1].i, (const float*)(uintptr_t)a[2].u, (const float*)(uintptr_t)a[3].u, (const float*)(uintptr_t)a[4].u, (float*)(uintptr_t)a[5].u, (float*)(uintptr_t)a[6].u, (int)a[7].i, (int)a[8].i, (int)a[9].i, stream);
+    case 43: return atmvfi_resize_bilinear_ac((const float*)(uintptr_t)a[0].u, (int64_t)a[1].i, (int64_t)a[2].i, (int64_t)a[3].i, (int64_t)a[4].i, (float*)(uintptr_t)a[5].u, (int)a[6].i, (int)a[7].i, (int)a[8].i, (int)a[9].i, (int)a[10].i, (int)a[11].i, (float)a[12].f, stream);
+    case 44: return atmvfi_rgb_to_yuv420((const void*)(uintptr_t)a[0].u, (int)a[1].i, (const float*)(uintptr_t)a[2].u, (int)a[3].i, (int)a[4].i, (int)a[5].i, (int)a[6].i, (int)a[7].i, (int)a[8].i, (int)a[9].i, (int)a[10].i, (int)a[11].i, (void*)(uintptr_t)a[12].u, stream);
+    case 45: return atmvfi_shutter_accumulate((int32_t*)(uintptr_t)a[0].u, (int)a[1].i, (int)a[2].i, (const float*)(uintptr_t)a[3].u, (int)a[4].i, (int)a[5].i, (int)a[6].i, (int)a[7].i, (const uint8_t*)(uintptr_t)a[8].u, (int)a[9].i, (int)a[10].i, (int)a[11].i, (int)a[12].i, stream);
+    case 46: return atmvfi_shutter_resolve((const int32_t*)(uintptr_t)a[0].u, (int)a[1].i, (int)a[2].i, (int)a[3].i, (int)a[4].i, (uint8_t*)(uintptr_t)a[5].u, (int)a[6].i, stream);
+    case 47: return atmvfi_split_planes((const float*)(uintptr_t)a[0].u, (int)a[1].i, (int64_t)a[2].i, (int)a[3].i, (const float*)(uintptr_t)a[4].u, (void*)(uintptr_t)a[5].u, (void*)(uintptr_t)a[6].u, (int)a[7].i, stream);
+    case 48: return atmvfi_split_planes_at((const float*)(uintptr_t)a[0].u, (int)a[1].i, (int64_t)a[2].i, (int)a[3].i, (const float*)(uintptr_t)a[4].u, (void*)(uintptr_t)a[5].u, (void*)(uintptr_t)a[6].u, (int)a[7].i, (int)a[8].i, (int)a[9].i, stream);
+    case 49: return atmvfi_ssim_psnr((const void*)(uintptr_t)a[0].u, (int64_t)a[1].i, (int64_t)a[2].i, (int64_t)a[3].i, (int64_t)a[4].i, (const float*)(uintptr_t)a[5].u, (int64_t)a[6].i, (int64_t)a[7].i, (int64_t)a[8].i, (int64_t)a[9].i, (int)a[10].i, (int)a[11].i, (int)a[12].i, (float)a[13].f, (int)a[14].i, (double*)(uintptr_t)a[15].u, (float*)(uintptr_t)a[16].u, (int64_t)a[17].i, stream);
+    case 50: return atmvfi_stem_fused((const float*)(uintptr_t)a[0].u, (int)a[1].i, (int)a[2].i, (int)a[3].i, (int)a[4].i, (int)a[5].i, (const void*)(uintptr_t)a[6].u, (const void*)(uintptr_t)a[7].u, (const float*)(uintptr_t)a[8].u, (const float*)(uintptr_t)a[9].u, (const void*)(uintptr_t)a[10].u, (const void*)(uintptr_t)a[11].u, (const float*)(uintptr_t)a[12].u, (const float*)(uintptr_t)a[13].u, (const void*)(uintptr_t)a[14].u, (const void*)(uintptr_t)a[15].u, (const float*)(uintptr_t)a[16].u, (const float*)(uintptr_t)a[17].u, (void*)(uintptr_t)a[18].u, (void*)(uintptr_t)a[19].u, (int64_t)a[20].i, stream);
+    case 51: return atmvfi_tta_merge((const float*)(uintptr_t)a[0].u, (const float*)(uintptr_t)a[1].u, (float*)(uintptr_t)a[2].u, (void*)(uintptr_t)a[3].u, (int)a[4].i, (int)a[5].i, (int)a[6].i, (int)a[7].i, (int)a[8].i, (int)a[9].i, (int)a[10].i, stream);
+    case 52: return atmvfi_warp_blend((const float*)(uintptr_t)a[0].u, (const float*)(uintptr_t)a[1].u, (const float*)(uintptr_t)a[2].u, (int)a[3].i, (int64_t)a[4].i, (float*)(uintptr_t)a[5].u, (float*)(uintptr_t)a[6].u, (float*)(uintptr_t)a[7].u, (float*)(uintptr_t)a[8].u, (float*)(uintptr_t)a[9].u, (float*)(uintptr_t)a[10].u, (float*)(uintptr_t)a[11].u, (const float*)(uintptr_t)a[12].u, (const float*)(uintptr_t)a[13].u, (float*)(uintptr_t)a[14].u, (int)a[15].i, (int)a[16].i, (int)a[17].i, (int)a[18].i, stream);
+    case 53: return atmvfi_warp_blend_planes((const float*)(uintptr_t)a[0].u, (const float*)(uintptr_t)a[1].u, (const float*)(uintptr_t)a[2].u, (int)a[3].i, (int64_t)a[4].i, (float*)(uintptr_t)a[5].u, (float*)(uintptr_t)a[6].u, (float*)(uintptr_t)a[7].u, (float*)(uintptr_t)a[8].u, (float*)(uintptr_t)a[9].u, (float*)(uintptr_t)a[10].u, (float*)(uintptr_t)a[11].u, (const float*)(uintptr_t)a[12].u, (const float*)(uintptr_t)a[13].u, (float*)(uintptr_t)a[14].u, (int)a[15].i, (void*)(uintptr_t)a[16].u, (void*)(uintptr_t)a[17].u, (int64_t)a[18].i, (int)a[19].i, (int)a[20].i, (int)a[21].i, (int)a[22].i, stream);
+    case 54: return atmvfi_warp_blend_tiled((const float*)(uintptr_t)a[0].u, (const float*)(uintptr_t)a[1].u, (const float*)(uintptr_t)a[2].u, (int)a[3].i, (int64_t)a[4].i, (float*)(uintptr_t)a[5].u, (float*)(uintptr_t)a[6].u, (float*)(uintptr_t)a[7].u, (float*)(uintptr_t)a[8].u, (float*)(uintptr_t)a[9].u, (float*)(uintptr_t)a[10].u, (float*)(uintptr_t)a[11].u, (const float*)(uintptr_t)a[12].u, (const float*)(uintptr_t)a[13].u, (float*)(uintptr_t)a[14].u, (int)a[15].i, (void*)(uintptr_t)a[16].u, (void*)(uintptr_t)a[17].u, (int64_t)a[18].i, (int)a[19].i, (int)a[20].i, (int)a[21].i, (int)a[22].i, stream);
+    case 55: return atmvfi_window_attention((const float*)(uintptr_t)a[0].u, (float*)(uintptr_t)a[1].u, (float*)(uintptr_t)a[2].u, (const int32_t*)(uintptr_t)a[3].u, (int)a[4].i, (int)a[5].i, (int)a[6].i, (int)a[7].i, (int)a[8].i, (int)a[9].i, (void*)(uintptr_t)a[10].u, (void*)(uintptr_t)a[11].u, (int)a[12].i, stream);
+    case 56: return atmvfi_window_attention_f16x3((const float*)(uintptr_t)a[0].u, (float*)(uintptr_t)a[1].u, (float*)(uintptr_t)a[2].u, (const int32_t*)(uintptr_t)a[3].u, (int)a[4].i, (int)a[5].i, (int)a[6].i, (int)a[7].i, (int)a[8].i, (int)a[9].i, (void*)(uintptr_t)a[10].u, (void*)(uintptr_t)a[11].u, (int)a[12].i, stream);
+    case 57: return atmvfi_window_attn_cross_motion((const float*)(uintptr_t)a[0].u, (float*)(uintptr_t)a[1].u, (float*)(uintptr_t)a[2].u, (const int32_t*)(uintptr_t)a[3].u, (int)a[4].i, (int)a[5].i, (int)a[6].i, (int)a[7].i, (int)a[8].i, stream);
+    case 58: return atmvfi_window_attn_self((const float*)(uintptr_t)a[0].u, (float*)(uintptr_t)a[1].u, (const int32_t*)(uintptr_t)a[2].u, (int)a[3].i, (int)a[4].i, (int)a[5].i, (int)a[6].i, (int)a[7].i, stream);
+    case 59: return atmvfi_yuv420_to_rgb((const void*)(uintptr_t)a[0].u, (int)a[1].i, (int)a[2].i, (int)a[3].i, (int)a[4].i, (int)a[5].i, (int)a[6].i, (void*)(uintptr_t)a[7].u, (int)a[8].i, (float*)(uintptr_t)a[9].u, (int)a[10].i, (int)a[11].i, (int)a[12].i, (int)a[13].i, stream);
+    case 60: return atmvfi_yuv420_window((const void*)(uintptr_t)a[0].u, (int)a[1].i, (int)a[2].i, (int)a[3].i, (int)a[4].i, (int)a[5].i, (int)a[6].i, (int)a[7].i, (int)a[8].i, (int)a[9].i, (int)a[10].i, (int)a[11].i, (float*)(uintptr_t)a[12].u, (int)a[13].i, (int)a[14].i, (int)a[15].i, (int)a[16].i, (void*)(uintptr_t)a[17].u, stream);
+    case 61: return atmvfi_yuv420p10_to_f32((const void*)(uintptr_t)a[0].u, (int)a[1].i, (int)a[2].i, (int)a[3].i, (int)a[4].i, (int)a[5].i, (int)a[6].i, (int)a[7].i, (int)a[8].i, (float*)(uintptr_t)a[9].u, (int)a[10].i, (int)a[11].i, (int)a[12].i, (int)a[13].i, stream);
+    case 62: return atmvfi_yuv_sub_decode((const void*)(uintptr_t)a[0].u, (int)a[1].i, (int)a[2].i, (int)a[3].i, (int)a[4].i, (int)a[5].i, (int)a[6].i, (int)a[7].i, (int)a[8].i, (int)a[9].i, (int64_t)a[10].i, (int64_t)a[11].i, (int64_t)a[12].i, (int)a[13].i, (int)a[14].i, (int)a[15].i, (int)a[16].i, (int)a[17].i, (void*)(uintptr_t)a[18].u, (int)a[19].i, (float*)(uintptr_t)a[20].u, (int)a[21].i, (int)a[22].i, (int)a[23].i, (int)a[24].i, stream);
+    case 63: return atmvfi_yuv_sub_encode((const void*)(uintptr_t)a[0].u, (int)a[1].i, (const float*)(uintptr_t)a[2].u, (int)a[3].i, (int)a[4].i, (int)a[5].i, (int)a[6].i, (int)a[7].i, (int)a[8].i, (int)a[9].i, (int)a[10].i, (int)a[11].i, (int)a[12].i, (int)a[13].i, (int)a[14].i, (int)a[15].i, (void*)(uintptr_t)a[16].u, stream);
+    case 64: return atmvfi_yuv_surface_decode((const void*)(uintptr_t)a[0].u, (int)a[1].i, (int)a[2].i, (int)a[3].i, (int)a[4].i, (int)a[5].i, (int)a[6].i, (int)a[7].i, (int)a[8].i, (int64_t)a[9].i, (int64_t)a[10].i, (int64_t)a[11].i, (int)a[12].i, (int)a[13].i, (int)a[14].i, (int)a[15].i, (int)a[16].i, (void*)(uintptr_t)a[17].u, (int)a[18].i, (float*)(uintptr_t)a[19].u, (int)a[20].i, (int)a[21].i, (int)a[22].i, (int)a[23].i, stream);
+    case 65: return atmvfi_yuv_surface_encode((const void*)(uintptr_t)a[0].u, (int)a[1].i, (const float*)(uintptr_t)a[2].u, (int)a[3].i, (int)a[4].i, (int)a[5].i, (int)a[6].i, (int)a[7].i, (int)a[8].i, (int)a[9].i, (int)a[10].i, (int)a[11].i, (int)a[12].i, (int)a[13].i, (int)a[14].i, (void*)(uintptr_t)a[15].u, stream);
     default: break;
     }
     atmvfi::set_error("plan_run: unknown function id %d", op->fn);
diff --git a/atm-vfi_amd/hip_ops.py b/atm-vfi_amd/hip_ops.py
--- a/atm-vfi_amd/hip_ops.py
+++ b/atm-vfi_amd/hip_ops.py
@@ -95,6 +95,8 @@
     "atmvfi_conv3x3_planes2": (c_i, [c_f, c_f, c_l, c_i, c_i, c_i, c_i, c_f, c_f, c_i, c_f, c_i, c_f, c_f, c_f, c_f, c_l, c_i, c_f, c_f, c_f, c_l, c_i, c_i, c_i, c_f]),
     "atmvfi_conv3x3_planes3": (c_i, [c_f, c_f, c_l, c_i, c_i, c_i, c_i, c_f, c_f, c_i, c_f, c_i, c_f, c_f, c_f, c_f, c_l, c_i, c_f, c_f, c_f, c_l, c_i, c_i, c_i, c_f, c_l, c_f]),
     "atmvfi_conv3x3_planes_workspace_floats": (c_l, [c_i, c_i, c_i, c_i, c_i]),
+    "atmvfi_conv3x3s2_planes_routed": (c_i, [c_i, c_i, c_i, c_i, c_i]),
+    "atmvfi_conv3x3s2_planes": (c_i, [c_f, c_f, c_l, c_f, c_f, c_l, c_i, c_i, c_i, c_i, c_i, c_f, c_f, c_i, c_f, c_i, c_f, c_f, c_f, c_f, c_l, c_i, c_f]),
     "atmvfi_conv3x3_planes_readout": (c_i, [c_f, c_f, c_l, c_i, c_i, c_i, c_i, c_f, c_f, c_i, c_f, c_f, c_f, c_f, c_l, c_f]),
     "atmvfi_refine_tail": (c_i, [c_f, c_l, c_f, c_f, c_f, c_f, c_f, c_i, c_i, c_i, c_f]),
     "atmvfi_layernorm": (c_i, [c_f, c_i, c_l, c_i, c_f, c_f, c_i, c_f, c_f, c_l, c_i, c_f, c_f, c_i, c_f]),
@@ -889,6 +891,44 @@
         p._srcs = (out, bias, prelu, ws)
         self._run("conv2d_split", meta, self.lib.atmvfi_conv2d, ctypes.byref(p), self._stream())
 
+    def conv3x3s2_routed(self, n: int, h: int, wd: int, w: PackedWeight) -> bool:
+        if self.precision != "f16x3" or w.hi is None or w.mode != GEMM_CONV or (w.kh, w.kw) != (3, 3) or self.gemm_tile_wn < 0:
+            return False
+        return bool(self.lib.atmvfi_conv3x3s2_planes_routed(n, h, wd, w.cin, w.cout))
+
+    def conv3x3s2_planes(self, x: Planes, n: int, h: int, wd: int, w: PackedWeight, out=None, bias=None, prelu=None,
+                         sink: Optional[Planes] = None, sink_c0: int = 0, in_chunk0: int = 0, x2: Optional[Planes] = None, x2_chunk0: int = 0,
+                         split_chunks: int = 0):
+        if self.precision != "f16x3" or w.hi is None or w.mode != GEMM_CONV or (w.kh, w.kw) != (3, 3):
+            raise ValueError("conv3x3s2_planes: needs the f16x3 engine and split 3x3 conv weights")
+        cin, cout = w.cin, w.cout
+        oh, ow = (h - 1) // 2 + 1, (wd - 1) // 2 + 1
+        c1 = 32 * split_chunks if x2 is not None else cin
+        for t, c0, cc, what in ((x, in_chunk0, c1, "x"),) + (((x2, x2_chunk0, cin - c1, "x2"),) if x2 is not None else ()):
+            if t.rows != n * h * wd or t.ld_rows <= t.rows or 32 * c0 + cc > t.chunks * 32:
+                raise ValueError(f"conv3x3s2_planes: {what} [{t.rows} (+{t.ld_rows - t.rows} spare), {t.c}] does not hold {n}x{h}x{wd} pixels x "
+                                 f"{cc} channels from chunk {c0} (one spare zero row is required)")
+        if x2 is not None and not 0 < 32 * split_chunks < cin:
+            raise ValueError("conv3x3s2_planes: split_chunks must cut the input channels at a 32-channel boundary inside (0, Cin)")
+        old = 0
+        if out is not None:
+            old, on, ooh, oow, oc = nhwc_view(out, "conv3x3s2_planes.out")
+            if (on, ooh, oow, oc) != (n, oh, ow, cout):
+                raise ValueError(f"conv3x3s2_planes: out {tuple(out.shape)} != [{n},{oh},{ow},{cout}]")
+        elif sink is None:
+            raise ValueError("conv3x3s2_planes: no output")
+        if sink is not None and (sink.rows != n * oh * ow or sink_c0 % 4 or sink_c0 + cout > sink.chunks * 32):
+            raise ValueError(f"conv3x3s2_planes: plane sink [{sink.rows},{sink.c}] cannot take {n * oh * ow} rows x {cout} channels at offset {sink_c0}")
+        meta = {"flops": 2.0 * n * oh * ow * cout * cin * 9, "bytes": 4.0 * (n * h * wd * cin + n * oh * ow * cout + cout * cin * 9),
+                "shape": f"M{n * oh * ow} N{cout} K{cin * 9}"}
+        off = in_chunk0 * x.ld_rows * 64
+        off2 = x2_chunk0 * x2.ld_rows * 64 if x2 is not None else 0
+        self._run("conv3x3s2_planes", meta, self.lib.atmvfi_conv3x3s2_planes, _ptr(x.t[0], off), _ptr(x.t[1], off), x.ld_rows,
+                  _ptr(x2.t[0], off2) if x2 is not None else None, _ptr(x2.t[1], off2) if x2 is not None else None,
+                  x2.ld_rows if x2 is not None else 0, split_chunks if x2 is not None else 0, n, h, wd, cin, _ptr(w.hi), _ptr(w.lo), cout,
+                  _ptr(out), old, _ptr(bias), _ptr(prelu), _ptr(sink.t[0]) if sink is not None else None,
+                  _ptr(sink.t[1]) if sink is not None else None, sink.ld_rows if sink is not None else 0, sink_c0, self._stream())
+
     def deconv(self, x, w: PackedWeight, out, bias=None, prelu=None, in_prelu=None, planes: Optional[Planes] = None,
                sink: Optional[Planes] = None, sink_c0: int = 0, in_shape=None):
         if x is None:
diff --git a/atm-vfi_amd/network.py b/atm-vfi_amd/network.py
--- a/atm-vfi_amd/network.py
+++ b/atm-vfi_amd/network.py
@@ -511,6 +511,10 @@
         else:
             wk, bias, prelu = f"pk:{p}.weight", P[f"{p}.bias"], None
         two = {} if src2 is None else {"x2": src2.p, "x2_chunk0": src2.chunk0, "split_chunks": src.c // 32}
+        if (stride, pad, dil) == (2, 1, 1) and P[wk].kh == 3 and hasattr(ops, "conv3x3s2_routed") and ops.conv3x3s2_routed(src.n, src.h, src.w, P[wk]):
+            ops.conv3x3s2_planes(src.p, src.n, src.h, src.w, P[wk], out=out, bias=bias, prelu=prelu, sink=sink, sink_c0=sink_c0,
+                                 in_chunk0=src.chunk0, **two)
+            return
         ops.conv_planes(src.p, src.n, src.h, src.w, P[wk], out=out, stride=stride, pad=pad, dil=dil, bias=bias, prelu=prelu, sink=sink,
                         sink_c0=sink_c0, in_chunk0=src.chunk0, **two)
 
diff --git a/include/atmvfi.h b/include/atmvfi.h
--- a/include/atmvfi.h
+++ b/include/atmvfi.h
@@ -97,6 +97,11 @@
                            const void* w_lo, int Cout, float* out, int out_ld, const float* bias, const float* prelu, void* out_hi,
                            void* out_lo, int64_t plane_rows, int out_c0, const float* plane_prelu, void* out_hi2, void* out_lo2,
                            int64_t plane_rows2, int out_c02, int out_cmin, int wn, float* workspace, int64_t workspace_floats, void* stream);
+int atmvfi_conv3x3s2_planes_routed(int N, int H, int W, int Cin, int Cout);
+int atmvfi_conv3x3s2_planes(const void* in_hi, const void* in_lo, int64_t in_rows, const void* in_hi2, const void* in_lo2,
+                            int64_t in_rows2, int split_chunks, int N, int H, int W, int Cin, const void* w_hi, const void* w_lo,
+                            int Cout, float* out, int out_ld, const float* bias, const float* prelu, void* out_hi, void* out_lo,
+                            int64_t plane_rows, int out_c0, void* stream);
 int atmvfi_layernorm(const float* in, int in_ld, int64_t in_gstride, int in_rpg,
                      const int32_t* src_row_map, float* out, int out_ld,
                      const float* gamma, const float* beta, int64_t rows, int C,
```

After: 51.87 (median of 6 runs). No clear change (+0.9%).
